# DARYL-GWZ/Proud-SLAM

Measured on AMD Instinct MI355X. Metric: rays/sec render+backward, Replica room0, 64 samples/ray, 1/2/4/8 MI355X, higher is better.
Workload: dtype f32

## Files before the change

### include/psvo.h

```cpp
#ifndef PSVO_H
#define PSVO_H

#include <stdint.h>

#ifdef __cplusplus
extern "C" {
#endif

enum {
    PSVO_OK = 0,
    PSVO_E_INVALID = 1,
    PSVO_E_LAUNCH = 2,
    PSVO_E_OVERFLOW = 3,
    PSVO_E_BUSY = 4,
    PSVO_E_SYSTEM = 5
};

const char *psvo_last_error(void);
const char *psvo_version(void);


int psvo_svo_intersect(void *stream, int b, int n, int m, float voxelsize, int n_max, const float *ray_start,
                       const float *ray_dir, const float *points, const int *children, int *idx, float *min_depth,
                       float *max_depth);
// ... 180 lines not shown
                          float voxel_size, int *table, int *row);
int psvo_mesh_depth_points(void *stream, int64_t n, const float *depth, const float *dirs, const float *pose,
                           double *out);
int64_t psvo_mesh_downsample_workspace_bytes(int64_t n);
int psvo_mesh_points_downsample(void *stream, int64_t n, const double *points, double cell, void *workspace,
                                double *out, int64_t *count);
int psvo_mesh_points_status(int64_t word);
int64_t psvo_mesh_ball_workspace_bytes(int64_t m);
int psvo_mesh_ball_any(void *stream, int64_t m, const double *points, int64_t n_verts, const float *verts,
                       double radius, void *workspace, uint8_t *hit, int64_t *status);

int psvo_adam_mark_rows(void *stream, int64_t m, const int *leaf, const int *vertex_idx, uint8_t *flags);
int psvo_adam_flags_from_state(void *stream, int64_t n_rows, const float *exp_avg, const float *exp_avg_sq,
                               uint8_t *flags);
int psvo_adam_step(void *stream, int n_tensors, float *const *params, const float *const *grads,
                   float *const *exp_avg, float *const *exp_avg_sq, const int64_t *numel, double lr, double beta1,
                   double beta2, double eps, double weight_decay, int64_t step);

typedef struct psvo_engine psvo_engine;

typedef struct psvo_map_desc {
    int64_t n_nodes;
    const float *centres;
    const int *structure;
    const int *vertex_idx;
    float *emb;
    int64_t n_emb;
    float *emb_m, *emb_v;
    float *dec[10];
    float *dec_m[10];
    float *dec_v[10];
    int width;
    float voxel_size, step_size, max_distance, truncation, max_depth;
    float w_rgb, w_depth, w_fs, w_sdf;
    double lr_emb, lr_dec, beta1, beta2, eps;
    float *grad_flat;
    const void *packed;
    uint8_t *emb_row_flags;
    uint8_t *emb_row_local;
} psvo_map_desc;

enum { PSVO_STEP_NO_ADAM = 1, PSVO_STEP_NO_LOSS = 4 };

int64_t psvo_map_grad_floats(int64_t n_emb);
int64_t psvo_map_grad_floats_w(int64_t n_emb, int width);

typedef struct psvo_pixel_frame {
    const float *dirs;
    const float *rgb;
    const float *depth;
    uint8_t *mask;
} psvo_pixel_frame;
int64_t psvo_sample_pixels_workspace_ints(int n_frames, int64_t n_pix);
int psvo_sample_pixels(void *stream, int n_frames, int64_t n_pix, int64_t k, const float *weights, int joint_sum,
                       const float *u, uint64_t seed, const psvo_pixel_frame *frames, int *workspace, int64_t *idx,
                       float *out_dirs, float *out_rgb, float *out_depth);

int64_t psvo_rows_workspace_ints(int64_t n_rows);
int psvo_rows_compact(void *stream, int64_t n_rows, int width, const float *grad, int *workspace, int *ids,
                      float *rows, int *count);
int psvo_rows_scatter_add(void *stream, int64_t n_list, int width, const int *ids, const float *rows, float *grad);
int psvo_rows_compact_flagged(void *stream, int64_t n_rows, int width, const float *grad, const uint8_t *flags,
                              int *workspace, int *ids, float *rows, int *count);
int psvo_rows_clear(void *stream, int64_t n_list, int width, const int *ids, float *grad, uint8_t *flags);
int psvo_rows_mark(void *stream, int64_t n_list, const int *ids, uint8_t *flags);
int psvo_rows_flags_from_grad(void *stream, int64_t n_rows, int width, const float *grad, uint8_t *flags);

psvo_engine *psvo_engine_new(void);
void psvo_engine_free(psvo_engine *e);
enum { PSVO_XCH_GATHER_I32 = 1, PSVO_XCH_SUM_I32 = 2, PSVO_XCH_SUM_F64 = 3, PSVO_XCH_QUERY = 0x100 };
typedef int (*psvo_exchange_fn)(void *user, int op, int64_t in_off, int64_t out_off, int64_t count, void *stream);
int64_t psvo_engine_exchange_words(int world, int64_t max_rays_global, int64_t max_rays_rank);
int psvo_engine_set_exchange(psvo_engine *e, int rank, int world, int64_t max_rays_global, int64_t max_rays_rank,
                             psvo_exchange_fn fn, void *user, int *xi32, double *xf64);

int psvo_engine_queued(psvo_engine *e);
int psvo_map_discard(psvo_engine *e);

enum {
    PSVO_PATH_QUERY_SPLIT = 1,
    PSVO_PATH_PADDED = 2,
    PSVO_PATH_DENSE_DECODER = 4,
    PSVO_PATH_INTERP_PASS = 8,
    PSVO_PATH_BWD_TWO_LAUNCH = 16
};
int psvo_engine_set_paths(psvo_engine *e, int paths);

int psvo_engine_select_stats(psvo_engine *e, void *stream, int64_t *out, int reset);

int psvo_engine_gate_stream(psvo_engine *e, void *stream);

int psvo_debug_set_lookback(int mask, int spin_bound, int delay_us);
int psvo_debug_set_bwd_split(int cost_a, int cost_b, int cost_b0);
int psvo_debug_bwd_split(int64_t units_a, int64_t units_b, int n_wg);
int psvo_debug_lb_helps(int64_t *out3, int reset);
int psvo_debug_set_pixel_draw(int mode);
int psvo_debug_select_samples(void *stream, int64_t r_hit, int s_max, float truncation, float max_depth,
                              const int *offsets, const int *ray_ns, const float *z_vals, int z_stride,
                              const int *rank_ray, const float *gt_depth, const float *sdf_s, const float *feat,
                              const int *leaf, const float *t, const int *ray_of, int64_t cap, int split, int *cidx,
                              int *offa, int *offb, float *feat_c, int *leaf_c, float *t_c, int *ray_of_c,
                              float *rgb_c, int *src_c, int *counts, uint64_t *desc, uint32_t tag, int *host_flag);
int64_t psvo_debug_select_granules(int64_t r_hit);
int psvo_debug_trunk_interp(void *stream, int fused, int64_t m_cap, const int *m_dev, const int *leaf, const float *t,
                            const int *ray_of, const int *ray_index, const float *rays_o, const float *rays_d,
                            const float *centres, const int *vertex_idx, const float *emb, float voxel_size,
                            const float *w1, const float *b1, const float *w2, const float *b2, const float *w3,
                            const float *b3, const float *w4, const float *b4, const float *w5, const float *b5,
                            float *images, float *sdf, float *h2, float *feat);
int psvo_debug_composite_loss(void *stream, int64_t r_hit, int s_max, float truncation, float max_depth,
                              const int *offsets, const int *ray_ns, const float *z_vals, int z_stride,
                              const int *rank_ray, const float *gt_rgb, const float *gt_depth, const float *sdf_s,
                              const float *rgb_s, const float *coef, float *workspace, float *color, float *depth,
                              float *grad_sdf_s, float *grad_rgb_s, int partials, const int *cidx);

enum { PSVO_TIME_MLP_FWD = 0, PSVO_TIME_MLP_BWD = 1, PSVO_TIME_INTERP_FWD = 2, PSVO_TIME_INTERP_BWD = 3,
       PSVO_TIME_INTERSECT = 4, PSVO_TIME_SAMPLE = 5, PSVO_TIME_POINTS = 6, PSVO_TIME_SELECT = 7,
       PSVO_TIME_REGIONS = 8 };
int psvo_engine_set_timing(psvo_engine *e, int on);
int psvo_engine_timing(psvo_engine *e, double *mean_ms);
int psvo_engine_set_clock(psvo_engine *e, int max_steps);
int psvo_engine_clock(psvo_engine *e, double *period_ms, int *n_steps);
int psvo_host_wait_stats(double *wait_us, long long *calls, long long *waited, int reset);

int psvo_map_query(psvo_engine *e, void *stream, const psvo_map_desc *d, int64_t n_rays, const float *rays_o,
                   const float *rays_d, uint64_t seed);
int psvo_map_step(psvo_engine *e, void *stream, const psvo_map_desc *d, int64_t n_rays, const float *rays_o,
                  const float *rays_d, const float *gt_rgb, const float *gt_depth, uint64_t seed, int64_t adam_step,
                  int flags, float *loss_out, int *stats_out);

typedef struct psvo_map_frames {
    int n_frames;
    int64_t rays_per_frame;
    const float *dirs_cam;
    float *poses, *pose_m, *pose_v;
    const int64_t *pose_step;
    double lr_pose;
    float *pose_grad;
    const float *next_dirs_cam;
    uint64_t next_seed;
    void *next_stream;
    const float *next_gt_depth;
} psvo_map_frames;
int psvo_map_step_frames(psvo_engine *e, void *stream, const psvo_map_desc *d, const psvo_map_frames *frames,
                         const float *gt_rgb, const float *gt_depth, const float *noise, uint64_t seed,
                         int64_t adam_step, int flags, float *loss_out, int *stats_out);

enum { PSVO_TRACK_DEPTH_FILTER = 2 };
int psvo_track_step(psvo_engine *e, void *stream, const psvo_map_desc *d, int64_t n_rays, const float *dirs_cam,
                    const float *gt_rgb, const float *gt_depth, float *pose, float *pose_m, float *pose_v, double lr,
                    const float *noise, uint64_t seed, int64_t adam_step, int flags, float *pose_grad,
                    float *loss_out, int *stats_out);

enum { PSVO_ADAM_ROWS_EXCHANGED = 1 };
int psvo_map_adam(psvo_engine *e, void *stream, const psvo_map_desc *d, int64_t adam_step);
int psvo_map_adam_ex(psvo_engine *e, void *stream, const psvo_map_desc *d, int64_t adam_step, int flags);
int psvo_map_join(psvo_engine *e, void *stream);
int psvo_map_side_wait(psvo_engine *e, void *stream);
int psvo_engine_grad_rays(psvo_engine *e, void *stream, int64_t n_rays, float *grad_o, float *grad_d);

typedef struct psvo_render_opts {
    int64_t tile_rays;
    int flags;
} psvo_render_opts;
enum { PSVO_RENDER_QUERY_ONLY = 1 };
enum {
    PSVO_RENDER_STAT_R_HIT = 0,
    PSVO_RENDER_STAT_P = 1,
    PSVO_RENDER_STAT_MAX_STEPS = 2,
// ... 78 lines not shown
```

### proud-slam_amd/csrc/composite.hip

```cpp
#include <hip/hip_runtime.h>

#include "lookback.h"
#include "psvo_common.h"
#include "query.h"
#include "select_common.h"

namespace psvo {
namespace {

__device__ __forceinline__ float wsum(float v) {
#pragma unroll
    for (int s = 32; s > 0; s >>= 1) v += __shfl_xor(v, s, 64);
    return v;
}
__device__ __forceinline__ int wmin(int v) {
#pragma unroll
    for (int s = 32; s > 0; s >>= 1) v = min(v, __shfl_xor(v, s, 64));
    return v;
}
__device__ __forceinline__ float sigm(float x) { return 1.0f / (1.0f + expf(-x)); }

__device__ __forceinline__ float comp_gw3(float gdp, float z, float gwx, bool has_c, float c0, float c1, float c2,
                                          float gr, float gg, float gb) {
    const float g = fmaf(gdp, z, gwx);
    return has_c ? fmaf(gb, c2, fmaf(gg, c1, fmaf(gr, c0, g))) : g;
}
__device__ __forceinline__ float comp_gw(float gdp, float z, float gwx, const float *c, float gr, float gg, float gb) {
    return c ? comp_gw3(gdp, z, gwx, true, c[0], c[1], c[2], gr, gg, gb) : comp_gw3(gdp, z, gwx, false, 0.f, 0.f,
                                                                                   0.f, gr, gg, gb);
}
__device__ __forceinline__ float comp_gsdf_sig(float gw, float dot, float tot, bool keep, float sp, float sn, float tr,
                                               float g) {
    const float gu = keep ? (gw - dot) / tot : 0.f;
    const float du = sp * sn * (sn - sp) / tr;
    return fmaf(gu, du, g);
}
__device__ __forceinline__ float comp_gsdf(float gw, float dot, float tot, bool keep, float sdf, float tr, float g) {
    const float a = sdf / tr;
    return comp_gsdf_sig(gw, dot, tot, keep, sigm(a), sigm(-a), tr, g);
}

__global__ __launch_bounds__(256) void k_composite_fwd(int64_t r_hit, int s_max, float tr,
                                                       const int *__restrict__ offsets,
                                                       const int *__restrict__ ray_ns,
                                                       const float *__restrict__ z_vals,
                                                       const float *__restrict__ sdf_s,
                                                       const float *__restrict__ rgb_s, float *__restrict__ sdf,
                                                       float *__restrict__ weights, float *__restrict__ color,
                                                       float *__restrict__ depth, float *__restrict__ z_min_out) {
    const int lane = threadIdx.x & 63;
    const int64_t r = (int64_t)blockIdx.x * (blockDim.x >> 6) + (threadIdx.x >> 6);
    if (r >= r_hit) return;
    const int off = offsets[r], ns = ray_ns[r];
    const float *z = z_vals + r * s_max;
    float *sd = sdf + r * s_max;
    float *wt = weights + r * s_max;
    int first = s_max;
    for (int s = lane; s < s_max; s += 64) {
        const float v = s < ns ? sdf_s[off + s] : 1.0f;
        sd[s] = v;
        if (s + 1 < s_max) {
            const float v1 = (s + 1) < ns ? sdf_s[off + s + 1] : 1.0f;
            if (v1 * v < 0.0f) first = min(first, s);
        }
    }
    first = wmin(first);
    const int ind = first == s_max ? 0 : first;
    const float zmin = z[ind];
    float tot = 0.f;
    for (int s = lane; s < s_max; s += 64) {
        const float v = sd[s];
        const float a = v / tr;
        float w = sigm(a) * sigm(-a);
        const bool keep = (z[s] < zmin + tr) && (s < ns);
        w = keep ? w : 0.0f;
        wt[s] = w;
        tot += w;
    }
    tot = wsum(tot) + 1e-8f;
    float cr = 0.f, cg = 0.f, cb = 0.f, dd = 0.f;
    for (int s = lane; s < s_max; s += 64) {
        const float w = wt[s] / tot;
        wt[s] = w;
        if (s < ns) {
            const float *c = rgb_s + (int64_t)(off + s) * 3;
            cr += w * c[0];
            cg += w * c[1];
            cb += w * c[2];
        }
        dd += w * z[s];
    }
    cr = wsum(cr);
    cg = wsum(cg);
    cb = wsum(cb);
    dd = wsum(dd);
    if (lane == 0) {
        color[r * 3 + 0] = cr;
        color[r * 3 + 1] = cg;
        color[r * 3 + 2] = cb;
        depth[r] = dd;
        if (z_min_out) z_min_out[r] = zmin;
    }
}

__global__ __launch_bounds__(256) void k_composite_bwd(int64_t r_hit, int s_max, float tr,
                                                       const int *__restrict__ offsets,
                                                       const int *__restrict__ ray_ns,
                                                       const float *__restrict__ z_vals,
                                                       const float *__restrict__ sdf,
                                                       const float *__restrict__ weights,
                                                       const float *__restrict__ rgb_s,
                                                       const float *__restrict__ g_color,
                                                       const float *__restrict__ g_depth,
                                                       const float *__restrict__ g_weights,
                                                       const float *__restrict__ g_sdf,
                                                       float *__restrict__ g_sdf_s, float *__restrict__ g_rgb_s) {
    const int lane = threadIdx.x & 63;
    const int64_t r = (int64_t)blockIdx.x * (blockDim.x >> 6) + (threadIdx.x >> 6);
    if (r >= r_hit) return;
    const int off = offsets[r], ns = ray_ns[r];
    const float *z = z_vals + r * s_max;
    const float *sd = sdf + r * s_max;
    const float *wt = weights + r * s_max;
    const float gr = g_color ? g_color[r * 3 + 0] : 0.f;
    const float gg = g_color ? g_color[r * 3 + 1] : 0.f;
    const float gb = g_color ? g_color[r * 3 + 2] : 0.f;
    const float gdp = g_depth ? g_depth[r] : 0.f;
    float dot = 0.f, tot = 0.f;
    for (int s = lane; s < s_max; s += 64) {
        const float gw = comp_gw(gdp, z[s], g_weights ? g_weights[r * s_max + s] : 0.f,
                                 s < ns ? rgb_s + (int64_t)(off + s) * 3 : nullptr, gr, gg, gb);
        dot = fmaf(gw, wt[s], dot);
    }
    dot = wsum(dot);
    int first = s_max;
    for (int s = lane; s < s_max; s += 64) {
        if (s + 1 < s_max && sd[s + 1] * sd[s] < 0.0f) first = min(first, s);
    }
    first = wmin(first);
    const float zmin = z[first == s_max ? 0 : first];
    for (int s = lane; s < s_max; s += 64) {
        const float a = sd[s] / tr;
        const bool keep = (z[s] < zmin + tr) && (s < ns);
        tot += keep ? sigm(a) * sigm(-a) : 0.f;
    }
    tot = wsum(tot) + 1e-8f;
    for (int s = lane; s < ns; s += 64) {
        const float *c = rgb_s + (int64_t)(off + s) * 3;
        const float W = wt[s];
        const float gw = comp_gw(gdp, z[s], g_weights ? g_weights[r * s_max + s] : 0.f, c, gr, gg, gb);
        g_sdf_s[off + s] = comp_gsdf(gw, dot, tot, z[s] < zmin + tr, sd[s], tr, g_sdf ? g_sdf[r * s_max + s] : 0.f);
        float *gc = g_rgb_s + (int64_t)(off + s) * 3;
        gc[0] = W * gr;
        gc[1] = W * gg;
        gc[2] = W * gb;
    }
}

constexpr int kPartColor = 0, kPartDepth = 1, kPartQFs = 5, kPartQSdf = 6, kPartN = 8;

struct CritTerms {
    float f, sm, xfs, ysdf;
};
__device__ __forceinline__ CritTerms crit_terms(float z, float p, float d, float tr, float max_depth) {
#pragma clang fp contract(off)
    CritTerms o;
    o.f = z < (d - tr) ? 1.0f : 0.0f;
    const float b = z > (d + tr) ? 1.0f : 0.0f;
    const float dm = (d > 0.0f && d < max_depth) ? 1.0f : 0.0f;
    o.sm = (1.0f - o.f) * (1.0f - b) * dm;
    o.xfs = p * o.f - o.f;
    o.ysdf = (z + p * tr) * o.sm - d * o.sm;
    return o;
}
__device__ __forceinline__ float crit_sq_add(float acc, float x) {
#pragma clang fp contract(off)
    return acc + x * x;
}
__device__ __forceinline__ float crit_grad(float cfs, float csdf, const CritTerms &t) {
#pragma clang fp contract(off)
    return cfs * t.xfs * t.f + csdf * t.ysdf * t.sm;
}

template <int J>
__global__ __launch_bounds__(256) void k_composite_loss(int64_t r_hit, int s_max, float tr, float max_depth,
                                                        const int *__restrict__ offsets,
                                                        const int *__restrict__ ray_ns,
                                                        const float *__restrict__ z_vals, int z_stride,
                                                        const int *__restrict__ rank_ray,
                                                        const float *__restrict__ gt_rgb,
                                                        const float *__restrict__ gt_depth,
                                                        const float *__restrict__ sdf_s,
                                                        const float *__restrict__ rgb_s,
                                                        const float *__restrict__ coef, float *__restrict__ part,
                                                        float *__restrict__ color, float *__restrict__ depth,
                                                        float *__restrict__ g_sdf_s, float *__restrict__ g_rgb_s,
                                                        int partials, const int *__restrict__ cidx) {
    const int lane = threadIdx.x & 63;
    const int64_t r = (int64_t)blockIdx.x * (blockDim.x >> 6) + (threadIdx.x >> 6);
    if (r >= r_hit) return;
    const int64_t orig = rank_ray[r];
    const int off = offsets[r], ns = ray_ns[r];
    const int lim = ns < s_max ? ns : s_max;
    const float d = gt_depth[orig];
    const float gt0 = gt_rgb[orig * 3 + 0], gt1 = gt_rgb[orig * 3 + 1], gt2 = gt_rgb[orig * 3 + 2];
    const float ccol = coef[0], cdep = coef[1], cfs = coef[2], csdf = coef[3];
    const float *z = z_vals + r * z_stride;
    auto z_at = [&](int s) { return s < ns ? z[s] : kMaxDepthFill; };
    auto sdf_at = [&](int s) { return s < ns ? sdf_s[off + s] : 1.0f; };
    auto ci_at = [&](int s) { return s < ns ? (cidx ? cidx[off + s] : off + s) : -1; };
    constexpr int JR = J > 0 ? J : 1;
    float zr[JR], pr[JR], c0r[JR], c1r[JR], c2r[JR];
    if constexpr (J > 0) {
#pragma unroll
        for (int j = 0; j < J; ++j) {
            const int s = lane + 64 * j;
            zr[j] = s < s_max ? z_at(s) : 0.f;
            pr[j] = sdf_at(s);
            const int ci = ci_at(s);
            const bool v = ci >= 0;
            const float *c = rgb_s + (int64_t)(v ? ci : 0) * 3;
            c0r[j] = v ? c[0] : 0.f;
            c1r[j] = v ? c[1] : 0.f;
            c2r[j] = v ? c[2] : 0.f;
        }
    }
    auto Z = [&](int j, int s) {
        if constexpr (J > 0) return zr[j]; else return z_at(s);
    };
    auto P = [&](int j, int s) {
        if constexpr (J > 0) return pr[j]; else return sdf_at(s);
    };
    auto C = [&](int j, int s, int k) {
        if constexpr (J > 0) return k == 0 ? c0r[j] : (k == 1 ? c1r[j] : c2r[j]);
        else {
            const int ci = ci_at(s);
            return ci >= 0 ? rgb_s[(int64_t)ci * 3 + k] : 0.f;
        }
    };
#define PSVO_FOR_S(lim) for (int j = 0, s = lane; (J == 0 || j < J) && s < (lim); ++j, s += 64)
    float pn[JR];
    if constexpr (J > 0) {
#pragma unroll
        for (int j = 0; j < J; ++j) {
            const float dn = __shfl_down(pr[j], 1, 64);
            const float nx = __shfl(pr[j + 1 < J ? j + 1 : j], 0, 64);
            pn[j] = lane < 63 ? dn : nx;
        }
    }
    int first = s_max;
    PSVO_FOR_S(lim) {
        const float v = P(j, s);
        float v1;
        if constexpr (J > 0) v1 = pn[j];
        else v1 = s + 1 < s_max ? sdf_at(s + 1) : 0.f;
        if (s + 1 < s_max && v1 * v < 0.0f) first = min(first, s);
    }
    first = wmin(first);
    const float zmin = z_at(first == s_max ? 0 : first);
    float spr[JR], snr[JR], wr[JR];
#pragma unroll
    for (int j = 0; j < JR; ++j) spr[j] = snr[j] = wr[j] = 0.f;
    float tot = 0.f;
    PSVO_FOR_S(lim) {
        const float a = P(j, s) / tr;
        const float sp = sigm(a), sn = sigm(-a);
        float w = sp * sn;
        const bool keep = (Z(j, s) < zmin + tr) && (s < ns);
        tot += keep ? w : 0.0f;
        if constexpr (J > 0) {
            spr[j] = sp;
            snr[j] = sn;
            wr[j] = keep ? w : 0.0f;
        }
    }
    tot = wsum(tot) + 1e-8f;
    if constexpr (J > 0) {
#pragma unroll
        for (int j = 0; j < J; ++j) wr[j] = wr[j] / tot;
    }
    auto weight_at = [&](int j, int s) {
        if constexpr (J > 0) {
            return wr[j];
        } else {
            const float a = P(j, s) / tr;
            const float w = sigm(a) * sigm(-a);
            const bool keep = (Z(j, s) < zmin + tr) && (s < ns);
            return (keep ? w : 0.0f) / tot;
        }
    };
    float cr = 0.f, cg = 0.f, cb = 0.f, dd = 0.f;
    PSVO_FOR_S(lim) {
        const float w = weight_at(j, s);
        if (s < ns) {
            cr += w * C(j, s, 0);
            cg += w * C(j, s, 1);
            cb += w * C(j, s, 2);
        }
        dd += w * Z(j, s);
    }
    cr = wsum(cr);
    cg = wsum(cg);
    cb = wsum(cb);
    dd = wsum(dd);
    float qfs = 0.f, qsdf = 0.f;
    if (partials) {
        PSVO_FOR_S(s_max) {
            const CritTerms t = crit_terms(Z(j, s), P(j, s), d, tr, max_depth);
            qfs = crit_sq_add(qfs, t.xfs);
            qsdf = crit_sq_add(qsdf, t.ysdf);
        }
        qfs = wsum(qfs);
        qsdf = wsum(qsdf);
    }
    const float rgb[3] = {cr, cg, cb};
    const float gt[3] = {gt0, gt1, gt2};
    float gcol[3], ac = 0.f;
#pragma unroll
    for (int c = 0; c < 3; ++c) {
        const float e = gt[c] - rgb[c];
        ac += fabsf(e);
        gcol[c] = -ccol * (e > 0.0f ? 1.0f : (e < 0.0f ? -1.0f : 0.0f));
    }
    const bool valid = d > 0.01f && d < max_depth;
    const float ed = d - dd;
    const float gdp = valid ? -cdep * (ed > 0.0f ? 1.0f : (ed < 0.0f ? -1.0f : 0.0f)) : 0.0f;
    if (lane == 0) {
        color[r * 3 + 0] = cr;
        color[r * 3 + 1] = cg;
        color[r * 3 + 2] = cb;
        depth[r] = dd;
        if (partials) {
            float *o = part + r * kPartN;
            o[kPartColor] = ac;
            o[kPartDepth] = valid ? fabsf(ed) : 0.0f;
            o[kPartQFs] = qfs;
            o[kPartQSdf] = qsdf;
            o[7] = 0.0f;
        }
    }
    float dot = 0.f;
    PSVO_FOR_S(lim) {
        const bool v = s < ns;
        const float gw = comp_gw3(gdp, Z(j, s), 0.f, v, v ? C(j, s, 0) : 0.f, v ? C(j, s, 1) : 0.f,
                                  v ? C(j, s, 2) : 0.f, gcol[0], gcol[1], gcol[2]);
        dot = fmaf(gw, weight_at(j, s), dot);
    }
    dot = wsum(dot);
    PSVO_FOR_S(ns) {
        const float W = weight_at(j, s);
        const float zs = Z(j, s);
        const float gw = comp_gw3(gdp, zs, 0.f, true, C(j, s, 0), C(j, s, 1), C(j, s, 2), gcol[0], gcol[1], gcol[2]);
        const float p = P(j, s);
        const float gsdf = crit_grad(cfs, csdf, crit_terms(zs, p, d, tr, max_depth));
        const int gi = ci_at(s);
        if (gi < 0) continue;
        if constexpr (J > 0)
            g_sdf_s[gi] = comp_gsdf_sig(gw, dot, tot, zs < zmin + tr, spr[j], snr[j], tr, gsdf);
        else
            g_sdf_s[gi] = comp_gsdf(gw, dot, tot, zs < zmin + tr, p, tr, gsdf);
        float *gc = g_rgb_s + (int64_t)gi * 3;
        gc[0] = W * gcol[0];
        gc[1] = W * gcol[1];
        gc[2] = W * gcol[2];
    }
#undef PSVO_FOR_S
}


constexpr int kSelWaves = 8, kSelMaxRpw = 16;
struct SelectArgs {
    const float4 *feat;
    const int *leaf, *ray_of;
    const float *t;
    int *cidx;
    int *offa, *offb;
    float4 *feat_c;
    int *leaf_c, *ray_of_c;
    float *t_c;
    float *rgb_c;
    int *src_c;
    int64_t cap;
    int split;
    int *counts;
    unsigned long long *desc;
    uint32_t tag;
    LbCtl ctl;
    int *host_flag;
};

using sel::sel_zmin;

struct SelFlags {
    bool keep, comp;
};
__device__ __forceinline__ SelFlags sel_flags(float zs, float zmin, float d, float tr, float max_depth) {
#pragma clang fp contract(off)
    SelFlags o;
    o.comp = zs < zmin + tr;
    const bool f = zs < (d - tr);
    const bool b = zs > (d + tr);
    const bool dm = d > 0.0f && d < max_depth;
    o.keep = o.comp || f || (!b && dm);
    return o;
}

__device__ unsigned long long psvo_g_sel_helps;

__global__ __launch_bounds__(512) void k_select_samples(int64_t r_hit, int rpw, int s_max, float tr, float max_depth,
                                                        const int *__restrict__ offsets,
                                                        const int *__restrict__ ray_ns,
                                                        const float *__restrict__ z_vals, int z_stride,
                                                        const int *__restrict__ rank_ray,
                                                        const float *__restrict__ gt_depth,
                                                        const float *__restrict__ sdf_s, SelectArgs a) {
    __shared__ int s_na[kSelWaves * kSelMaxRpw], s_nb[kSelWaves * kSelMaxRpw];
    __shared__ int s_oa[kSelWaves * kSelMaxRpw], s_ob[kSelWaves * kSelMaxRpw];
    __shared__ float s_zmin[kSelWaves * kSelMaxRpw];
    __shared__ int s_nc[kSelWaves], s_base[2];
    const int lane = threadIdx.x & 63, w = threadIdx.x >> 6;
    const int blk = (int)blockIdx.x;
    lb_debug_delay(a.ctl, blk);
    if (threadIdx.x == 0) lb_mark_started<3>(a.desc, blk, (int)gridDim.x, a.tag);
    const int64_t r0 = ((int64_t)blk * kSelWaves + w) * rpw;
    const uint64_t below = (1ull << lane) - 1ull;
    const bool split = a.split != 0;
    auto count_classes = [&](int cur) {
        const int64_t c0 = ((int64_t)cur * kSelWaves + w) * rpw;
        int nc_w = 0;
        for (int k = 0; k < rpw; ++k) {
            const int64_t r = c0 + k;
            int na = 0, nb = 0;
            float zmin = 0.f;
            if (r < r_hit) {
                const int off = offsets[r], ns = ray_ns[r];
                const float *z = z_vals + r * z_stride;
                const float d = gt_depth[rank_ray[r]];
                zmin = sel_zmin(lane, s_max, ns, off, z, sdf_s);
                for (int s0 = 0; s0 < ns; s0 += 64) {
                    const int s = s0 + lane;
                    SelFlags f{false, false};
                    if (s < ns) f = sel_flags(z[s], zmin, d, tr, max_depth);
                    const int nk = __popcll(__ballot(f.keep)), nc = __popcll(__ballot(f.comp && s < ns));
                    na += split ? nc : nk;
                    nb += split ? nk - nc : 0;
                    nc_w += nc;
                }
            }
            if (lane == 0) {
                s_na[w * rpw + k] = na;
                s_nb[w * rpw + k] = nb;
// ... 109 lines not shown
            a.offa[r] = ba;
            if (split) a.offb[r] = bb;
        }
        for (int s0 = 0; s0 < ns; s0 += 64) {
            const int s = s0 + lane;
            SelFlags f{false, false};
            if (s < ns) f = sel_flags(z[s], zmin, d, tr, max_depth);
            const bool in_a = split ? (f.comp && s < ns) : f.keep;
            const bool in_b = split && f.keep && !f.comp;
            const uint64_t bal_a = __ballot(in_a), bal_b = __ballot(in_b);
            const int64_t j = in_a ? (int64_t)(ba + __popcll(bal_a & below))
                                   : a.cap + bb + __popcll(bal_b & below);
            if (s < ns) a.cidx[off + s] = (in_a || in_b) ? (int)j : -1;
            if (in_a || in_b) {
                const int64_t src = off + s;
                a.leaf_c[j] = a.leaf[src];
                a.t_c[j] = a.t[src];
                a.ray_of_c[j] = a.ray_of[src];
                if (a.src_c) a.src_c[j] = (int)src;
                if (a.feat_c) {
#pragma unroll
                    for (int q = 0; q < 4; ++q) a.feat_c[j * 4 + q] = a.feat[src * 4 + q];
                }
                if (in_b) {
#pragma unroll
                    for (int k = 0; k < 3; ++k) a.rgb_c[j * 3 + k] = 0.f;
                }
            }
            ba += __popcll(bal_a);
            bb += __popcll(bal_b);
        }
    }
}

}
}

using namespace psvo;

extern "C" int psvo_composite_fwd(void *stream, int64_t r_hit, int s_max, float truncation, const int *offsets,
                                  const int *ray_ns, const float *z_vals, const float *sdf_s, const float *rgb_s,
                                  float *sdf, float *weights, float *color, float *depth, float *z_min) {
    PSVO_REQUIRE(r_hit >= 0 && s_max > 0 && truncation > 0.f, "composite_fwd: bad sizes");
    if (r_hit == 0) return PSVO_OK;
    psvo::launch(k_composite_fwd, dim3(div_up(r_hit, 4)), dim3(256), 0, as_stream(stream), r_hit, s_max,
                       truncation, offsets, ray_ns, z_vals, sdf_s, rgb_s, sdf, weights, color, depth, z_min);
    return check_launch("composite_fwd");
}

extern "C" int psvo_composite_bwd(void *stream, int64_t r_hit, int s_max, float truncation, const int *offsets,
                                  const int *ray_ns, const float *z_vals, const float *sdf, const float *weights,
                                  const float *rgb_s, const float *grad_color, const float *grad_depth,
                                  const float *grad_weights, const float *grad_sdf, float *grad_sdf_s,
                                  float *grad_rgb_s) {
    PSVO_REQUIRE(r_hit >= 0 && s_max > 0 && truncation > 0.f, "composite_bwd: bad sizes");
    if (r_hit == 0) return PSVO_OK;
    psvo::launch(k_composite_bwd, dim3(div_up(r_hit, 4)), dim3(256), 0, as_stream(stream), r_hit, s_max,
                       truncation, offsets, ray_ns, z_vals, sdf, weights, rgb_s, grad_color, grad_depth,
                       grad_weights, grad_sdf, grad_sdf_s, grad_rgb_s);
    return check_launch("composite_bwd");
}


extern "C" int psvo_composite_loss(void *stream, int64_t r_hit, int s_max, float truncation, float max_depth,
                                   const int *offsets, const int *ray_ns, const float *z_vals, const int *rank_ray,
                                   const float *gt_rgb, const float *gt_depth, const float *sdf_s,
                                   const float *rgb_s, const float *coef, float *workspace, float *color,
                                   float *depth, float *grad_sdf_s, float *grad_rgb_s) {
    return psvo::composite_loss_z(stream, r_hit, s_max, truncation, max_depth, offsets, ray_ns, z_vals, s_max,
                                  rank_ray, gt_rgb, gt_depth, sdf_s, rgb_s, coef, workspace, color, depth, grad_sdf_s,
                                  grad_rgb_s, true, nullptr);
}

int psvo::composite_loss_z(void *stream, int64_t r_hit, int s_max, float truncation, float max_depth,
                           const int *offsets, const int *ray_ns, const float *z_vals, int z_stride,
                           const int *rank_ray, const float *gt_rgb, const float *gt_depth, const float *sdf_s,
                           const float *rgb_s, const float *coef, float *workspace, float *color, float *depth,
                           float *grad_sdf_s, float *grad_rgb_s, bool partials, const int *cidx) {
    PSVO_REQUIRE(r_hit >= 0 && s_max > 0 && truncation > 0.f && z_stride >= s_max, "composite_loss: bad sizes");
    PSVO_REQUIRE(offsets && ray_ns && z_vals && rank_ray && gt_rgb && gt_depth && sdf_s && rgb_s && coef &&
                     workspace && color && depth && grad_sdf_s && grad_rgb_s,
                 "composite_loss: null pointer");
    if (r_hit == 0) return PSVO_OK;
    auto kern = s_max <= 128   ? k_composite_loss<2>
                : s_max <= 256 ? k_composite_loss<4>
                : s_max <= 512 ? k_composite_loss<8>
                               : k_composite_loss<0>;
    psvo::launch(kern, dim3(div_up(r_hit, 4)), dim3(256), 0, as_stream(stream), r_hit, s_max, truncation,
                       max_depth, offsets, ray_ns, z_vals, z_stride, rank_ray, gt_rgb, gt_depth, sdf_s, rgb_s, coef,
                       workspace, color, depth, grad_sdf_s, grad_rgb_s, partials ? 1 : 0, cidx);
    return check_launch("composite_loss");
}

int psvo::select_samples(hipStream_t st, int64_t r_hit, int s_max, float truncation, float max_depth,
                         const int *offsets, const int *ray_ns, const float *z_vals, int z_stride, const int *rank_ray,
                         const float *gt_depth, const float *sdf_s, const float *feat, const int *leaf, const float *t,
                         const int *ray_of, int64_t cap, bool split, int *cidx, int *offa, int *offb, float *feat_c,
                         int *leaf_c, float *t_c, int *ray_of_c, float *rgb_c, int *src_c, int *counts,
                         unsigned long long *desc, uint32_t tag, int *host_flag) {
    PSVO_REQUIRE(r_hit >= 0 && s_max > 0 && truncation > 0.f && z_stride >= s_max && tag != 0 && cap > 0,
                 "select_samples: bad sizes");
    PSVO_REQUIRE(!split || (offb != nullptr && rgb_c != nullptr),
                 "select_samples: the split needs class B's offsets and colour rows");
    const int rpw = select_rays_per_wave(r_hit);
    PSVO_REQUIRE(rpw <= kSelMaxRpw, "select_samples: %lld hit rays exceed the selection's %d",
                 (long long)r_hit, kSelWaves * kSelMaxRpw * kLbMaxBlocks);
    if (r_hit == 0) return PSVO_OK;
    SelectArgs a{reinterpret_cast<const float4 *>(feat), leaf, ray_of, t, cidx, offa, offb,
                 reinterpret_cast<float4 *>(feat_c), leaf_c, ray_of_c, t_c, rgb_c, src_c, cap, split ? 1 : 0, counts, desc, tag,
                 lb_ctl(4), host_flag};
    psvo::launch(k_select_samples, dim3(div_up(r_hit, (int64_t)kSelWaves * rpw)), dim3(64 * kSelWaves), 0, st, r_hit,
                 rpw, s_max, truncation, max_depth, offsets, ray_ns, z_vals, z_stride, rank_ray, gt_depth, sdf_s, a);
    return check_launch("select_samples");
}

int psvo::lb_helps_select(int64_t *out1, bool reset) {
    unsigned long long h = 0;
    if (hipDeviceSynchronize() != hipSuccess || hipMemcpyFromSymbol(&h, HIP_SYMBOL(psvo_g_sel_helps), sizeof(h)) != hipSuccess)
        return set_error(PSVO_E_LAUNCH, "debug_lb_helps: copy failed");
    *out1 = (int64_t)h;
    const unsigned long long z = 0;
    if (reset && hipMemcpyToSymbol(HIP_SYMBOL(psvo_g_sel_helps), &z, sizeof(z)) != hipSuccess)
        return set_error(PSVO_E_LAUNCH, "debug_lb_helps: reset failed");
    return PSVO_OK;
}

int psvo::select_rays_per_wave(int64_t r_hit) {
    const int64_t per = (int64_t)kSelWaves * kLbMaxBlocks;
    return r_hit <= per ? 1 : (int)((r_hit + per - 1) / per);
}

int64_t psvo::select_granules(int64_t r_hit) {
    return lb_granules<3>(div_up(r_hit, (int64_t)kSelWaves * select_rays_per_wave(r_hit)));
}
```

### proud-slam_amd/csrc/engine.cpp

```cpp
#include <stdio.h>
#include <stdlib.h>
#include <string.h>

#include <utility>

#include "engine_internal.h"

namespace psvo {
RenderWs *&engine_render_ws(psvo_engine *e) { return e->render; }
bool engine_data_parallel(const psvo_engine *e) { return e->x.on(); }
}

using namespace psvo;
using namespace psvo::eng;

namespace psvo {
thread_local KernelClock *g_kclock = nullptr;

namespace eng {

void *arena_buf(Arena &a, hipStream_t st, int slot, size_t bytes, int *rc) {
    if (bytes == 0) bytes = 16;
    if (a.cap[slot] >= bytes) return a.p[slot];
    if (a.p[slot]) {
// ... 143 lines not shown
        return set_error(PSVO_E_LAUNCH, "engine: aux stream creation failed");
    for (hipEvent_t *ev : evs)
        if (hipEventCreateWithFlags(ev, (ev == &e->dfeat_ready ? 0 : hipEventDisableTiming) |
                                            hipEventDisableSystemFence) != hipSuccess)
            return set_error(PSVO_E_LAUNCH, "engine: event creation failed");
    return PSVO_OK;
}

void dec_sizes(int W, int64_t (&n)[10]) {
    const int64_t w = W;
    const int64_t v[10] = {w * 16, w, w * w, w, 129 * w, 129, w * 144, w, 3 * w, 3};
    for (int i = 0; i < 10; ++i) n[i] = v[i];
}

int map_adam(hipStream_t st, const psvo_map_desc *d, float *grads, int64_t adam_step, const PoseAdam *pa,
             bool sparse_rows) {
    constexpr int kMax = 11 + kXchMaxFrames;
    float *p[kMax];
    const float *g[kMax];
    float *m[kMax], *v[kMax];
    int64_t n[kMax], steps[kMax];
    double lr[kMax];
    int zero[kMax];
    const uint8_t *rows[kMax] = {};
    if (sparse_rows) rows[0] = d->emb_row_flags;
    p[0] = d->emb;
    g[0] = grads;
    m[0] = d->emb_m;
    v[0] = d->emb_v;
    n[0] = d->n_emb * 16;
    lr[0] = d->lr_emb;
    zero[0] = 1;
    int64_t off = d->n_emb * 16;
    int64_t kDecSizes[10];
    dec_sizes(d->width, kDecSizes);
    for (int i = 0; i < 10; ++i) {
        p[1 + i] = d->dec[i];
        g[1 + i] = grads + off;
        m[1 + i] = d->dec_m[i];
        v[1 + i] = d->dec_v[i];
        n[1 + i] = kDecSizes[i];
        lr[1 + i] = d->lr_dec;
        zero[1 + i] = 0;
        off += kDecSizes[i];
    }
    int cnt = 11;
    for (int i = 0; i < cnt; ++i) steps[i] = adam_step;
    for (int f = 0; pa && f < pa->n; ++f, ++cnt) {
        p[cnt] = pa->p[f];
        g[cnt] = pa->g[f];
        m[cnt] = pa->m[f];
        v[cnt] = pa->v[f];
        n[cnt] = 6;
        lr[cnt] = pa->lr;
        zero[cnt] = 0;
        steps[cnt] = pa->step[f];
    }
    return adam_launch(st, cnt, p, g, m, v, n, lr, d->beta1, d->beta2, d->eps, 0.0, adam_step, zero, steps, rows);
}

int pose_adam(hipStream_t st, const psvo_map_desc *d, const PoseAdam &pa) {
    if (pa.n == 0) return PSVO_OK;
    int64_t n6[kXchMaxFrames];
    double lr[kXchMaxFrames];
    int zero[kXchMaxFrames];
    for (int k = 0; k < pa.n; ++k) {
        n6[k] = 6;
        lr[k] = pa.lr;
        zero[k] = 0;
    }
    return adam_launch(st, pa.n, pa.p, pa.g, pa.m, pa.v, n6, lr, d->beta1, d->beta2, d->eps, 0.0, 1, zero,
                       const_cast<int64_t *>(pa.step));
}

}
}

extern "C" psvo_engine *psvo_engine_new(void) {
    psvo_engine *e = new psvo_engine();
    const char *ipass = getenv("PSVO_INTERP_PASS");
    if (ipass && ipass[0] == '1') e->paths |= PSVO_PATH_INTERP_PASS;
    const char *two = getenv("PSVO_BWD_TWO_LAUNCH");
    if (two && two[0] == '1') e->paths |= PSVO_PATH_BWD_TWO_LAUNCH;
    for (auto &q : e->qs)
        if (query_set_init(q) != PSVO_OK) {
            psvo_engine_free(e);
            return nullptr;
        }
    return e;
}

static EngineExchange exchange_layout(int world, int64_t max_rays_global, int64_t max_rays_rank) {
    EngineExchange x;
    x.world = world;
    x.nch = dist_slot0_rows(max_rays_global) / kSamplerG;
    x.max_rays_rank = max_rays_rank > 0 ? max_rays_rank : max_rays_global;
    x.cw = dist_count_words((int)x.max_rays_rank);
    return x;
}

extern "C" int64_t psvo_engine_exchange_words(int world, int64_t max_rays_global, int64_t max_rays_rank) {
    if (world < 1 || max_rays_global < 1 || max_rays_rank < 0 || max_rays_rank > max_rays_global) return -1;
    const EngineExchange x = exchange_layout(world, max_rays_global, max_rays_rank);
    return x.table_off() + x.table_words();
}

extern "C" int psvo_engine_set_exchange(psvo_engine *e, int rank, int world, int64_t max_rays_global,
                                        int64_t max_rays_rank, psvo_exchange_fn fn, void *user, int *xi32,
                                        double *xf64) {
    PSVO_REQUIRE(e, "engine_set_exchange: null engine");
    PSVO_REQUIRE(world >= 1 && rank >= 0 && rank < world && max_rays_global >= 1 && max_rays_rank >= 0 &&
                     max_rays_rank <= max_rays_global,
                 "engine_set_exchange: bad rank %d / world %d / max_rays_global %lld / max_rays_rank %lld", rank,
                 world, (long long)max_rays_global, (long long)max_rays_rank);
    PSVO_REQUIRE(e->q_count == 0, "engine_set_exchange: queries are queued");
    PSVO_REQUIRE(!fn || (xi32 && xf64), "engine_set_exchange: exchange buffers required");
    e->x = exchange_layout(world, max_rays_global, max_rays_rank);
    e->x.fn = fn;
    e->x.user = user;
    e->x.rank = rank;
    e->x.xi32 = xi32;
    e->x.xf64 = xf64;
    return PSVO_OK;
}

extern "C" int psvo_engine_set_paths(psvo_engine *e, int paths) {
    PSVO_REQUIRE(e && (paths & ~(PSVO_PATH_QUERY_SPLIT | PSVO_PATH_PADDED | PSVO_PATH_DENSE_DECODER |
                               PSVO_PATH_INTERP_PASS | PSVO_PATH_BWD_TWO_LAUNCH)) == 0,
                 "engine_set_paths: bad arguments");
    PSVO_REQUIRE(e->q_count == 0, "engine_set_paths: queries are queued");
    e->paths = paths;
    return PSVO_OK;
}

extern "C" int psvo_engine_gate_stream(psvo_engine *e, void *stream) {
    PSVO_REQUIRE(e, "engine_gate_stream: null engine");
    e->draw_gate_used = true;
    if (!e->draw_gate_recorded) return PSVO_OK;
    return st_wait(as_stream(stream), e->draw_gate_ev, "engine_gate_stream");
}

extern "C" int psvo_engine_select_stats(psvo_engine *e, void *stream, int64_t *out, int reset) {
    PSVO_REQUIRE(e && out, "engine_select_stats: null argument");
    for (int i = 0; i < 5; ++i) out[i] = 0;
    if (!e->a.p[kSelCnt]) return PSVO_OK;
    hipStream_t st = as_stream(stream);
    int c[psvo::kSelCountInts];
    if (hipMemcpyAsync(c, e->a.p[kSelCnt], sizeof(c), hipMemcpyDeviceToHost, st) != hipSuccess ||
        hipStreamSynchronize(st) != hipSuccess)
        return set_error(PSVO_E_LAUNCH, "engine_select_stats: copy failed");
    unsigned long long u[3];
    memcpy(u, c + 4, sizeof(u));
    out[0] = (int64_t)c[0] + c[1];
    out[1] = c[3];
    out[2] = (int64_t)u[0];
    out[3] = (int64_t)u[1];
    out[4] = (int64_t)u[2];
    if (c[2] & psvo::kLbFlagTimeout) {
        ENG_CALL(zero_async(static_cast<int *>(e->a.p[kSelCnt]) + 2, sizeof(int), st, "engine_select_stats"));
        if (e->host_flags) *(volatile int *)e->host_flags = 0;
        e->sel_zero_gen = 0;
        return set_error(PSVO_E_LAUNCH, "engine_select_stats: a sample selection's look-back wait was abandoned");
    }
    if (reset)
        ENG_CALL(zero_async(static_cast<int *>(e->a.p[kSelCnt]) + 4, 6 * sizeof(int), st, "engine_select_stats"));
    return PSVO_OK;
}

extern "C" int psvo_engine_set_timing(psvo_engine *e, int on) {
    PSVO_REQUIRE(e, "engine_set_timing: null engine");
    EngineTimer &t = e->tm;
    const char *mk = getenv("PSVO_TIMING_MARKERS");
    if (on && !t.ev[0][0])
        for (int r = 0; r < PSVO_TIME_REGIONS; ++r)
            for (int k = 0; k < 2; ++k)
                if (hipEventCreateWithFlags(&t.ev[r][k], hipEventReleaseToDevice) != hipSuccess)
                    return set_error(PSVO_E_LAUNCH, "engine_set_timing: hipEventCreate failed");
    const unsigned kc_flags = hipEventReleaseToDevice;
    if (on && !t.kc.ev[0][0])
        for (int i = 0; i < psvo::KernelClock::kMax; ++i)
            for (int k = 0; k < 2; ++k)
                if (hipEventCreateWithFlags(&t.kc.ev[i][k], kc_flags) != hipSuccess)
                    return set_error(PSVO_E_LAUNCH, "engine_set_timing: hipEventCreate failed");
    timer_collect(e, true);
    if (psvo::g_kclock == &t.kc) psvo::g_kclock = nullptr;
    t.kc.depth = 0;
    t.kc.overflow = false;
    t.on = on != 0;
    t.overlap = on == 2;
    t.markers = mk && *mk == '1';
    const char *ks = getenv("PSVO_TIMING_SPAN");
    t.kc.sum = !(ks && *ks == '1');
    t.kc.n = 0;
    t.kc.n_inst = 0;
    for (int r = 0; r < PSVO_TIME_REGIONS; ++r) {
        t.ms[r] = 0.0;
        t.n[r] = 0;
        t.kms[r] = 0.0;
        t.starts[r] = 0;
    }
    return PSVO_OK;
}

extern "C" int psvo_engine_timing(psvo_engine *e, double *mean_ms) {
    PSVO_REQUIRE(e && mean_ms, "engine_timing: null argument");
    EngineTimer &t = e->tm;
    timer_collect(e, true);
    for (int r = 0; r < PSVO_TIME_REGIONS; ++r) {
        if (t.markers)
            mean_ms[r] = t.n[r] ? t.ms[r] / (double)t.n[r] : -1.0;
        else
// ... 114 lines not shown
```

### proud-slam_amd/csrc/engine_internal.h

```cpp
#pragma once

#include <hip/hip_runtime.h>
#include <stdint.h>
#include <time.h>

#include <vector>

#include "psvo_common.h"
#include "lookback.h"
#include "query.h"

namespace psvo {

enum QSlot { kStats, kHitIdx, kHitT0, kHitT1, kRayNv, kRayDsum, kRayRank, kRankRay, kSIdx, kSDepth, kSDist, kRayNs,
             kOffsets, kBlkOut, kRayCnt, kCoefQ, kLbDesc, kLeafQ, kTQ, kRayOfQ, kDistSums, kMDev, kNvRank, kCol0Rank,
             kQSlots };
enum Slot {
    kLeaf, kT, kRayOf, kZ, kMask, kFeat, kImages, kSdfS, kRgbS, kAct, kMasks, kSdf, kWeights, kColor,
    kDepth, kZmin, kCritWs, kSums, kGLoss, kGColor, kGDepth, kGSdf, kGSdfS, kGRgbS, kMlpWs, kDfeat, kDecGrad,
    kGradEmb, kGradOD, kRaysO, kRaysD, kDTmp, kPoseGrad, kSumsC, kCoef, kIbWs,
    kCidx, kOffB, kFeatB, kLeafB, kTB, kRayOfB, kSdfB, kSelCnt, kSelDesc,
    kOffB2, kH2, kSrcC, kSlots
};

// ... 23 lines not shown
    const float *ro = nullptr, *rd = nullptr;
    const float *dirs = nullptr;
    const float *counts_gt = nullptr;
    uint64_t seed = 0;
    int max_steps = 0;
    hipEvent_t p1 = nullptr;
    hipEvent_t done2 = nullptr;
    bool p2_pending = false;
    const float *p2_gt = nullptr;
    float p2_tr = 0.f, p2_max_depth = 0.f;
};

}

struct EngineTimer {
    bool on = false;
    bool overlap = false;
    bool pending = false;
    bool markers = false;
    unsigned used = 0;
    hipEvent_t ev[PSVO_TIME_REGIONS][2] = {};
    double ms[PSVO_TIME_REGIONS] = {};
    int64_t n[PSVO_TIME_REGIONS] = {};
    psvo::KernelClock kc;
    double kms[PSVO_TIME_REGIONS] = {};
    int64_t starts[PSVO_TIME_REGIONS] = {};
};

struct EngineExchange {
    psvo_exchange_fn fn = nullptr;
    void *user = nullptr;
    int rank = 0, world = 1;
    int nch = 1;
    int cw = 8;
    int64_t max_rays_rank = 0;
    int *xi32 = nullptr;
    double *xf64 = nullptr;
    bool on() const { return fn != nullptr; }
    int64_t in_off() const { return 0; }
    int64_t all_off() const { return cw; }
    int64_t q2_in_off() const { return all_off() + (int64_t)world * cw; }
    int64_t q2_all_off() const { return q2_in_off() + psvo::kDistWordsPerRank; }
    int64_t table_off() const { return (q2_all_off() + (int64_t)world * psvo::kDistWordsPerRank + 63) / 64 * 64; }
    int64_t table_words() const { return (int64_t)psvo::kSamplerG * nch; }
    int call(int op, int64_t in, int64_t out, int64_t count, hipStream_t st, const char *what) const {
        const int rc = fn(user, op, in, out, count, st);
        if (rc != 0) return psvo::set_error(PSVO_E_LAUNCH, "exchange (%s) failed with %d", what, rc);
        return PSVO_OK;
    }
};

struct EngineClock {
    std::vector<hipEvent_t> ev;
    int n = 0;
    bool on = false;
};

struct psvo_engine {
    EngineExchange x;
    EngineClock clk;
    psvo::Arena a;
    psvo::QuerySet qs[2];
    int q_head = 0, q_count = 0;
    uint32_t lb_tag = 0;
    hipStream_t side = nullptr;
    hipStream_t q2s = nullptr;
    hipEvent_t in_ready = nullptr;
    hipStream_t aux = nullptr;
    hipStream_t lossq = nullptr;
    hipEvent_t dfeat_ready = nullptr, emb_done = nullptr, z_ready = nullptr, coef_ready = nullptr,
               grads_ready = nullptr, prep_fork = nullptr, prep_done = nullptr, loss_done = nullptr;
    hipEvent_t adam_done = nullptr;
    bool bwd_recorded = false;
    bool adam_pending = false;
    hipEvent_t next_ready = nullptr;
    hipEvent_t draw_gate = nullptr;
    hipEvent_t draw_gate_ev = nullptr;
    bool draw_gate_recorded = false;
    bool draw_gate_used = false;
    EngineTimer tm;
    bool images_next = false;
    const float *images_w0 = nullptr;
    int paths = 0;
    int64_t m_early = 0;
    uint32_t sel_tag = 0;
    uint32_t sel_zero_gen = 0;
    int *host_flags = nullptr;
    bool grads_clean = false;
    const float *clean_buf = nullptr;
    psvo::RenderWs *render = nullptr;
};

#define ENG_CALL(x)                     \
    do {                                \
        const int _rc = (x);            \
        if (_rc != PSVO_OK) return _rc; \
    } while (0)

#define ENG_BUF(T, name, slot, bytes)                                              \
    T *name = reinterpret_cast<T *>(arena_buf(e->a, st, slot, (bytes), &rc));     \
    if (!name) return rc;
#define Q_BUF(T, name, slot, bytes)                                              \
    T *name = reinterpret_cast<T *>(arena_buf(q.a, st, slot, (bytes), &rc));    \
    if (!name) return rc;

#pragma GCC visibility push(hidden)
namespace psvo {
namespace eng {

inline int ev_record(hipEvent_t ev, hipStream_t st, const char *who) {
    if (hipEventRecord(ev, st) == hipSuccess) return PSVO_OK;
    return set_error(PSVO_E_LAUNCH, "%s: event record failed", who);
}
inline int st_wait(hipStream_t st, hipEvent_t ev, const char *who) {
    if (hipStreamWaitEvent(st, ev, 0) == hipSuccess) return PSVO_OK;
    return set_error(PSVO_E_LAUNCH, "%s: stream wait failed", who);
}
inline int zero_async(void *p, size_t bytes, hipStream_t st, const char *who) {
    if (hipMemsetAsync(p, 0, bytes, st) == hipSuccess) return PSVO_OK;
    return set_error(PSVO_E_LAUNCH, "%s: memset failed", who);
}
inline int fork_join(hipStream_t from, hipStream_t st, hipEvent_t ev) {
    if (from == st) return PSVO_OK;
    ENG_CALL(ev_record(ev, from, "engine"));
    return st_wait(st, ev, "engine");
}

inline double now_ns() {
    timespec t;
    clock_gettime(CLOCK_MONOTONIC, &t);
    return t.tv_sec * 1e9 + t.tv_nsec;
}

void *arena_buf(Arena &a, hipStream_t st, int slot, size_t bytes, int *rc);
void timer_collect(psvo_engine *e, bool block = false);
void mark(psvo_engine *e, hipStream_t st, int region, int end);
int join_adam(psvo_engine *e, hipStream_t st, const char *who, double host_wait_us = 0.0);
inline bool engine_overlap(psvo_engine *e) { return !e->tm.on || e->tm.overlap; }
int ensure_aux(psvo_engine *e);
void dec_sizes(int W, int64_t (&n)[10]);
struct PoseAdam {
    int n = 0;
    float *p[kXchMaxFrames], *m[kXchMaxFrames], *v[kXchMaxFrames];
    const float *g[kXchMaxFrames];
    int64_t step[kXchMaxFrames];
    double lr = 0.0;
};
int map_adam(hipStream_t st, const psvo_map_desc *d, float *grads, int64_t adam_step, const PoseAdam *pa = nullptr,
             bool sparse_rows = false);
int pose_adam(hipStream_t st, const psvo_map_desc *d, const PoseAdam &pa);

int query_set_init(QuerySet &s);
void query_set_free(QuerySet &s);
void host_wait_report();
int query_enqueue(psvo_engine *e, hipStream_t st, QuerySet &q, const psvo_map_desc *d, int64_t R,
                  const float *rays_o, const float *rays_d, uint64_t seed, const char *who,
                  const float *noise = nullptr, bool record_done = true, const float *counts_gt = nullptr);
int take_query(psvo_engine *e, hipStream_t st, const psvo_map_desc *d, int64_t R, const float *rays_o,
               const float *rays_d, uint64_t seed, const char *who, QuerySet **out, const float *noise = nullptr,
               const float *counts_gt = nullptr);
int freed_wait(QuerySet &q, hipStream_t s);
int release_query(psvo_engine *e, hipStream_t st, QuerySet *q);
struct QueryGuard {
    psvo_engine *e;
    hipStream_t st;
    QuerySet *q = nullptr;
// ... 23 lines not shown
```

### proud-slam_amd/csrc/engine_step.cpp

```cpp
#include <stdint.h>
#include <string.h>

#include <algorithm>

#include "engine_internal.h"
#include "interp_load.h"

using namespace psvo;
using namespace psvo::eng;

namespace {

struct Samples {
    int *offsets = nullptr, *leaf = nullptr, *ray_of = nullptr;
    float *tt = nullptr, *feat = nullptr, *rgb_s = nullptr, *act = nullptr;
    uint64_t *masks = nullptr;
};

struct Render {
    int64_t r_hit = 0, m = 0;
    int s_max = 0;
    int *rank_ray = nullptr, *ray_rank = nullptr, *ray_ns = nullptr;
    float *z_vals = nullptr, *images = nullptr, *sdf_s = nullptr;
    Samples s;
// ... 302 lines not shown
    ENG_BUF(float, g_sdf, kGSdf, RS * sizeof(float));
    ENG_CALL(psvo_criterion_bwd_ex(stream, r_hit, s_max, d->truncation, d->max_depth, q.rank_ray, gt_rgb, gt_depth,
                                   q.color, q.depth, q.sdf, q.z_vals, loss_out, g_loss, dtmp, dthr, g_color, g_depth,
                                   g_sdf));
    ENG_BUF(float, g_sdf_s, kGSdfS, M * sizeof(float));
    ENG_BUF(float, g_rgb_s, kGRgbS, M * 3 * sizeof(float));
    ENG_CALL(psvo_composite_bwd(stream, r_hit, s_max, d->truncation, q.s.offsets, q.ray_ns, q.z_vals, q.sdf, q.weights,
                                q.s.rgb_s, g_color, g_depth, nullptr, g_sdf, g_sdf_s, g_rgb_s));
    *g_sdf_s_out = g_sdf_s;
    *g_rgb_s_out = g_rgb_s;
    return PSVO_OK;
}

int frames_update(psvo_engine *e, hipStream_t st, const psvo_map_desc *d, const psvo_map_frames *fr,
                  const Render &q, const float *grad_od, int64_t R, PoseAdam *pa) {
    int rc = PSVO_OK;
    float *pg = fr->pose_grad;
    if (!pg) {
        ENG_BUF(float, gbuf, kPoseGrad, (size_t)fr->n_frames * 8 * sizeof(float));
        pg = gbuf;
    }
    ENG_CALL(psvo::pose_grad_frames_rays(st, fr->n_frames, fr->rays_per_frame, q.ray_rank, fr->dirs_cam, grad_od,
                                         grad_od + R * 3, fr->poses, pg));
    pa->n = 0;
    pa->lr = fr->lr_pose;
    for (int f = 0; f < fr->n_frames; ++f) {
        if (fr->pose_step[f] < 1) continue;
        const int k = pa->n++;
        pa->p[k] = fr->poses + f * 6;
        pa->m[k] = fr->pose_m + f * 6;
        pa->v[k] = fr->pose_v + f * 6;
        pa->g[k] = pg + f * 8;
        pa->step[k] = fr->pose_step[f];
    }
    return PSVO_OK;
}

int frames_lookahead(psvo_engine *e, hipStream_t st, const psvo_map_desc *d, const psvo_map_frames *fr,
                     int64_t R, const Render &cur, const float *grad_od, bool record_done) {
    int rc = PSVO_OK;
    PSVO_REQUIRE(e->q_count == 0, "map_step_frames: a query is already queued");
    QuerySet &q = e->qs[e->q_head];
    ENG_CALL(freed_wait(q, st));
    ENG_BUF(float, rays_o, kRaysO, (size_t)R * 3 * sizeof(float));
    ENG_BUF(float, rays_d, kRaysD, (size_t)R * 3 * sizeof(float));
    float *pg = fr->pose_grad;
    if (!pg) {
        ENG_BUF(float, gbuf, kPoseGrad, (size_t)fr->n_frames * 8 * sizeof(float));
        pg = gbuf;
    }
    ENG_CALL(psvo::pose_step_frames(st, fr->n_frames, fr->rays_per_frame, cur.ray_rank, fr->dirs_cam,
                                    grad_od, grad_od + R * 3, fr->poses, fr->pose_m, fr->pose_v, fr->pose_step,
                                    fr->lr_pose, d->beta1, d->beta2, d->eps, pg, fr->next_dirs_cam, rays_o, rays_d));
    ENG_CALL(query_enqueue(e, st, q, d, R, rays_o, rays_d, fr->next_seed, "map_step_frames (look-ahead)", nullptr,
                           record_done, fr->next_gt_depth));
    q.dirs = fr->next_dirs_cam;
    q.pending = true;
    e->q_count++;
    return PSVO_OK;
}

struct MapStep {
    psvo_engine *e;
    hipStream_t st;
    const psvo_map_desc *d;
    const psvo_map_frames *fr;
    int flags;
    int64_t R, adam_step;
    const float *rays_o, *rays_d, *gt_rgb, *gt_depth;
    float *loss_out;
    bool overlap = false, dist = false, want_loss = false, wait_next = false, ahead = false, split = false;
    hipStream_t ax = nullptr, lq = nullptr, eb = nullptr;
    const float *counts_gt = nullptr;
    uint8_t *mark_into = nullptr;
    bool sparse_rows = false;
    QuerySet *qset = nullptr;
    Render q;
    bool empty = false;
    int64_t n_hit = 0;
    Samples k;
    int *cidx = nullptr, *sel_cnt = nullptr, *offb = nullptr;
    const int *h2_src = nullptr;
    float *crit_ws = nullptr, *coef = nullptr, *g_sdf_s = nullptr, *g_rgb_s = nullptr;
    double *sums = nullptr;
    float *grads = nullptr, *grad_od = nullptr;
    float *G[10] = {};

    bool two_class() const { return q.sparse && d->width == 128; }
    int64_t m_rows() const { return q.sparse ? 2 * q.m : q.m; }
    bool join_loss() const { return want_loss && lq != ax; }
    bool no_adam() const { return (flags & PSVO_STEP_NO_ADAM) != 0; }
};

int step_select(MapStep &s) {
    psvo_engine *e = s.e;
    hipStream_t st = s.st;
    const psvo_map_desc *d = s.d;
    const Render &q = s.q;
    s.k = q.s;
    if (!q.sparse || s.empty) return PSVO_OK;
    int rc = PSVO_OK;
    const int64_t M = q.m, r_hit = q.r_hit;
    const int64_t M2 = 2 * M;
    ENG_BUF(int, cx, kCidx, M * sizeof(int));
    ENG_BUF(int, offa, kOffB, (size_t)(r_hit + 1) * sizeof(int));
    float *feat_c = nullptr;
    if (!q.h2) {
        ENG_BUF(float, fc, kFeatB, M2 * 16 * sizeof(float));
        feat_c = fc;
    }
    ENG_BUF(int, leaf_c, kLeafB, M2 * sizeof(int));
    ENG_BUF(float, t_c, kTB, M2 * sizeof(float));
    ENG_BUF(int, ray_of_c, kRayOfB, M2 * sizeof(int));
    ENG_BUF(int, cnt, kSelCnt, psvo::kSelCountInts * sizeof(int));
    ENG_BUF(unsigned long long, desc, kSelDesc, (size_t)psvo::select_granules(r_hit) * sizeof(unsigned long long));
    if (e->sel_zero_gen != e->a.gen[kSelDesc]) {
        ENG_CALL(zero_async(desc, e->a.cap[kSelDesc], st, "map_step"));
        ENG_CALL(zero_async(cnt, psvo::kSelCountInts * sizeof(int), st, "map_step"));
        e->sel_zero_gen = e->a.gen[kSelDesc];
    }
    if (!e->host_flags) {
        if (hipHostMalloc(reinterpret_cast<void **>(&e->host_flags), sizeof(int),
                          hipHostMallocCoherent | hipHostMallocMapped) != hipSuccess)
            return set_error(PSVO_E_LAUNCH, "map_step: pinned allocation failed");
        *e->host_flags = 0;
    }
    if (s.two_class()) {
        ENG_BUF(int, ob, kOffB2, (size_t)(r_hit + 1) * sizeof(int));
        s.offb = ob;
    }
    ENG_BUF(float, rgb_c, kRgbS, M2 * 3 * sizeof(float));
    int *src_c = nullptr;
    if (q.h2) {
        ENG_BUF(int, sc, kSrcC, M2 * sizeof(int));
        src_c = sc;
    }
    e->sel_tag = e->sel_tag == 0xffffffffu ? 1u : e->sel_tag + 1u;
    mark(e, st, PSVO_TIME_SELECT, 0);
    if (e->draw_gate_used && !e->draw_gate &&
        hipEventCreateWithFlags(&e->draw_gate, hipEventDisableSystemFence) != hipSuccess)
        return set_error(PSVO_E_LAUNCH, "map_step: event creation failed");
    {
        psvo::StopBind gate(e->draw_gate_used ? e->draw_gate : nullptr, true);
        const int sel_rc = psvo::select_samples(st, r_hit, q.s_max, d->truncation, d->max_depth, q.s.offsets, q.ray_ns,
                                                q.z_vals, q.z_stride, q.rank_ray, s.gt_depth, q.sdf_s, q.s.feat,
                                                q.s.leaf, q.s.tt, q.s.ray_of, M, s.two_class(), cx, offa, s.offb,
                                                feat_c, leaf_c, t_c, ray_of_c, rgb_c, src_c, cnt, desc, e->sel_tag,
                                                e->host_flags);
        if (gate.consumed() && gate.bound()) {
            e->draw_gate_ev = gate.bound();
            e->draw_gate_recorded = true;
        }
        ENG_CALL(sel_rc);
    }
    mark(e, st, PSVO_TIME_SELECT, 1);
    ENG_BUF(float, sdf_b, kSdfB, M * sizeof(float));
    ENG_BUF(float, act, kAct, (size_t)psvo_mlp_act_floats(M, d->width) * sizeof(float));
    ENG_BUF(uint64_t, masks, kMasks, (size_t)psvo_mlp_mask_words(M, d->width) * sizeof(uint64_t));
    const psvo::H2Rows h2r{nullptr, q.h2, src_c};
    float *feat_k = src_c ? q.s.feat : feat_c;
    ENG_CALL(mlp_fwd_prepared(st, M, d->width, feat_k, q.images, sdf_b, rgb_c, act, masks, cnt,
                              src_c ? &h2r : nullptr));
    mark(e, st, PSVO_TIME_MLP_FWD, 1);
    s.k = Samples{offa, leaf_c, ray_of_c, t_c, feat_k, rgb_c, act, masks};
    s.h2_src = src_c;
    s.cidx = cx;
    s.sel_cnt = cnt;
    return PSVO_OK;
}

int step_normalisers(MapStep &s) {
    psvo_engine *e = s.e;
    hipStream_t st = s.st, ax = s.ax;
    const psvo_map_desc *d = s.d;
    const Render &q = s.q;
    QuerySet *qset = s.qset;
    const EngineExchange &x = e->x;
    int rc = PSVO_OK;
    ENG_BUF(float, crit_ws, kCritWs, psvo_criterion_workspace_floats(q.r_hit) * sizeof(float));
    s.crit_ws = crit_ws;
    double *sums_c = x.xf64;
    s.sums = x.xf64 ? x.xf64 + 8 : nullptr;
    if (!s.dist) {
        ENG_BUF(double, sc, kSumsC, 8 * sizeof(double));
        ENG_BUF(double, sl, kSums, 8 * sizeof(double));
        sums_c = sc;
        s.sums = sl;
    }
    const bool coef_q = !s.dist && s.counts_gt && qset->counts_gt == s.counts_gt;
    const bool sums_q = s.dist && s.counts_gt && qset->counts_gt != nullptr &&
                        !(qset->host_stats[PSVO_STAT_FLAGS] & psvo::PSVO_FLAG_UNION_UNCOUNTED);
    s.coef = coef_q ? static_cast<float *>(qset->a.p[kCoefQ]) : nullptr;
    if (!coef_q) {
        ENG_BUF(float, cbuf, kCoef, 4 * sizeof(float));
        s.coef = cbuf;
    }
    if (s.dist) {
        if (sums_q) {
            sums_c = static_cast<double *>(qset->a.p[kDistSums]);
            ENG_CALL(st_wait(ax, qset->done2, "map_step"));
        } else {
            ENG_CALL(criterion_counts(ax, s.empty ? 0 : q.r_hit, q.s_max, d->truncation, d->max_depth, q.rank_ray,
                                      s.gt_depth, q.z_vals, q.z_stride, q.z_stride == q.s_max ? nullptr : q.ray_ns,
                                      crit_ws, sums_c));
            ENG_CALL(x.call(PSVO_XCH_SUM_F64, 0, 0, 8, ax, "loss normalisers"));
        }
        ENG_CALL(criterion_coef_from_sums(ax, sums_c, s.n_hit, q.s_max, d->truncation, d->w_rgb, d->w_depth, d->w_fs,
                                          d->w_sdf, kCritFlags, s.coef));
    } else if (!coef_q) {
        ENG_CALL(psvo::criterion_coef_z(ax, q.r_hit, q.s_max, d->truncation, d->max_depth, q.rank_ray, s.gt_depth,
                                        q.z_vals, q.z_stride, q.ray_ns, d->w_rgb, d->w_depth, d->w_fs, d->w_sdf,
                                        kCritFlags, crit_ws, sums_c, s.coef));
    }
    if (!coef_q) ENG_CALL(fork_join(ax, st, e->coef_ready));
    if (s.mark_into && !s.empty && !psvo::mlp_bwd_fuses_interp(d->width))
        ENG_CALL(psvo_adam_mark_rows(ax, q.m, q.s.leaf, d->vertex_idx, s.mark_into));
    return PSVO_OK;
}

int step_loss(MapStep &s) {
    psvo_engine *e = s.e;
    hipStream_t st = s.st, lq = s.lq;
    const psvo_map_desc *d = s.d;
    const Render &q = s.q;
    int rc = PSVO_OK;
    ENG_BUF(float, color, kColor, (size_t)q.r_hit * 3 * sizeof(float));
    ENG_BUF(float, depth, kDepth, (size_t)q.r_hit * sizeof(float));
    ENG_BUF(float, g_sdf_s, kGSdfS, s.m_rows() * sizeof(float));
    ENG_BUF(float, g_rgb_s, kGRgbS, s.m_rows() * 3 * sizeof(float));
    s.g_sdf_s = g_sdf_s;
    s.g_rgb_s = g_rgb_s;
    if (!s.empty)
        ENG_CALL(psvo::composite_loss_z(st, q.r_hit, q.s_max, d->truncation, d->max_depth, q.s.offsets, q.ray_ns,
                                        q.z_vals, q.z_stride, q.rank_ray, s.gt_rgb, s.gt_depth, q.sdf_s, s.k.rgb_s,
                                        s.coef, s.crit_ws, color, depth, g_sdf_s, g_rgb_s, s.want_loss || s.dist,
                                        s.cidx));
    if (!s.want_loss) return PSVO_OK;
    ENG_CALL(fork_join(st, lq, e->grads_ready));
    if (!s.empty)
        ENG_CALL(psvo_criterion_reduce(lq, q.r_hit, s.crit_ws, s.sums));
    else
        ENG_CALL(zero_async(s.sums, 8 * sizeof(double), lq, "map_step"));
    if (s.dist) ENG_CALL(e->x.call(PSVO_XCH_SUM_F64, 8, 8, 8, lq, "loss sums"));
    ENG_CALL(psvo_criterion_finalize(lq, s.sums, s.n_hit, q.s_max, d->w_rgb, d->w_depth, d->w_fs, d->w_sdf,
                                     d->truncation, kCritFlags, s.loss_out));
    if (lq != s.ax) ENG_CALL(ev_record(e->loss_done, lq, "map_step"));
    return PSVO_OK;
}

int step_grad_buffers(MapStep &s) {
    psvo_engine *e = s.e;
    hipStream_t st = s.st;
    int rc = PSVO_OK;
    s.grads = s.d->grad_flat;
    if (!s.grads) {
        ENG_BUF(float, gbuf, kDecGrad, psvo_map_grad_floats_w(s.d->n_emb, s.d->width) * sizeof(float));
        s.grads = gbuf;
    }
    int64_t sizes[10];
    dec_sizes(s.d->width, sizes);
    int64_t off = s.d->n_emb * 16;
    for (int i = 0; i < 10; ++i) {
        s.G[i] = s.grads + off;
        off += sizes[i];
    }
    ENG_BUF(float, grad_od, kGradOD, (size_t)s.R * 6 * sizeof(float));
    s.grad_od = grad_od;
    return PSVO_OK;
}

int step_clock(psvo_engine *e, hipStream_t on) {
    if (e->clk.on && e->clk.n < (int)e->clk.ev.size()) ENG_CALL(ev_record(e->clk.ev[e->clk.n++], on, "map_step"));
    return PSVO_OK;
}

int step_empty(MapStep &s, QueryGuard &guard) {
    psvo_engine *e = s.e;
    ENG_CALL(fork_join(s.ax, s.st, e->emb_done));
    ENG_CALL(zero_async(s.grads, (size_t)psvo_map_grad_floats_w(s.d->n_emb, s.d->width) * sizeof(float), s.st,
                        "map_step"));
    e->grads_clean = false;
    ENG_CALL(guard.release());
    if (!s.no_adam()) ENG_CALL(map_adam(s.st, s.d, s.grads, s.adam_step));
    return step_clock(e, s.st);
}

int step_backward(MapStep &s) {
    psvo_engine *e = s.e;
    hipStream_t st = s.st, ax = s.ax, eb = s.eb;
    const psvo_map_desc *d = s.d;
    const Render &q = s.q;
    const Samples &k = s.k;
    int rc = PSVO_OK;
    const int64_t M = q.m, R = s.R;
    const int n_split = 256;
    ENG_BUF(float, mlp_ws, kMlpWs, psvo_mlp_workspace_floats_w(M, d->width, n_split) * sizeof(float));
    ENG_BUF(float, dfeat, kDfeat, M * 16 * sizeof(float));
    const bool fuse_ib = psvo::mlp_bwd_fuses_interp(d->width);
    float *grad_emb = s.grads;
    const size_t emb_bytes = (size_t)d->n_emb * 16 * sizeof(float);
    const bool emb_dirty = !(e->grads_clean && e->clean_buf == grad_emb);
    if (fuse_ib && emb_dirty) ENG_CALL(zero_async(grad_emb, emb_bytes, st, "map_step"));
    float *gx = nullptr;
    if (fuse_ib) {
        ENG_BUF(float, gxb, kIbWs, (size_t)s.m_rows() * 3 * sizeof(float));
        gx = gxb;
    }
    const psvo::InterpFuse ipf{k.leaf,  k.ray_of,      q.rank_ray, d->vertex_idx, k.tt, s.rays_o, s.rays_d, d->centres,
                               d->emb,  d->voxel_size, grad_emb,   gx,            s.mark_into};
    mark(e, st, PSVO_TIME_MLP_BWD, 0);
    const psvo::InterpFuse ipf_b{k.leaf + M, k.ray_of + M, q.rank_ray, d->vertex_idx, k.tt + M, s.rays_o, s.rays_d,
                                 d->centres, d->emb, d->voxel_size, grad_emb, gx ? gx + 3 * M : nullptr, s.mark_into};
    const psvo::TrunkBwd tbw{s.sel_cnt ? s.sel_cnt + 1 : nullptr, s.g_sdf_s + M, s.h2_src ? k.feat : k.feat + M * 16,
                             fuse_ib ? &ipf_b : nullptr, s.h2_src ? q.h2 : nullptr, s.h2_src ? s.h2_src + M : nullptr,
                             (e->paths & PSVO_PATH_BWD_TWO_LAUNCH) != 0};
    ENG_CALL(mlp_bwd(st, M, d->width, k.feat, q.images, k.rgb_s, k.act, k.masks, s.g_sdf_s, s.g_rgb_s, dfeat, s.G, 0,
                     n_split, mlp_ws, s.overlap ? e->dfeat_ready : nullptr, fuse_ib ? &ipf : nullptr,
                     s.split ? ax : nullptr, s.sel_cnt, s.two_class() ? &tbw : nullptr, s.h2_src));
    mark(e, st, PSVO_TIME_MLP_BWD, 1);
    if (s.overlap) e->bwd_recorded = true;
    if (s.overlap && eb != st) ENG_CALL(st_wait(eb, e->dfeat_ready, "map_step"));
    if (!fuse_ib && emb_dirty) ENG_CALL(zero_async(grad_emb, emb_bytes, eb, "map_step"));
    e->grads_clean = false;
    e->clean_buf = grad_emb;
    mark(e, eb, PSVO_TIME_INTERP_BWD, 0);
    if (fuse_ib) {
        ENG_CALL(psvo::interp_rays_gx(eb, q.r_hit, k.offsets, q.rank_ray, k.tt, gx, s.grad_od, s.grad_od + R * 3,
                                      s.two_class() ? s.offb : nullptr, s.two_class() ? k.tt + M : nullptr,
                                      s.two_class() ? gx + 3 * M : nullptr));
    } else {
        ENG_BUF(float, ib_ws2, kIbWs, psvo_interp_bwd_workspace_floats(q.r_hit, q.s_max) * sizeof(float));
        ENG_CALL(psvo_interp_bwd_chunked(eb, q.r_hit, q.s_max, 16, d->voxel_size, k.offsets, q.rank_ray, k.leaf, k.tt,
                                         s.rays_o, s.rays_d, d->centres, d->vertex_idx, d->emb, dfeat, grad_emb,
                                         s.grad_od, s.grad_od + R * 3, ib_ws2));
    }
    mark(e, eb, PSVO_TIME_INTERP_BWD, 1);
    if (s.overlap && eb != st) {
        ENG_CALL(ev_record(e->emb_done, eb, "map_step"));
        ENG_CALL(st_wait(st, e->emb_done, "map_step"));
    }
    if (s.join_loss()) ENG_CALL(st_wait(s.split ? ax : st, e->loss_done, "map_step"));
    return PSVO_OK;
}

int step_tail(MapStep &s) {
    psvo_engine *e = s.e;
    hipStream_t st = s.st, ax = s.ax, eb = s.eb;
    const psvo_map_desc *d = s.d;
    int rc = PSVO_OK;
    PoseAdam pa;
    if (s.ahead) {
        if (s.wait_next) ENG_CALL(st_wait(eb, e->next_ready, "map_step"));
        ENG_CALL(frames_lookahead(e, eb, d, s.fr, s.R, s.q, s.grad_od, eb != st));
    } else if (s.fr) {
        ENG_CALL(frames_update(e, st, d, s.fr, s.q, s.grad_od, s.R, &pa));
    }
    hipStream_t os = st;
    if (!s.no_adam()) {
        if (s.split) os = ax;
        ENG_CALL(map_adam(os, d, s.grads, s.adam_step, &pa, s.sparse_rows));
        e->grads_clean = true;
        if (s.ahead) {
            ENG_BUF(float, images, kImages, psvo_mlp_image_floats_w(d->width) * sizeof(float));
            ENG_CALL(mlp_images(os, d->width, d->dec, images));
            e->images_next = true;
            e->images_w0 = d->dec[0];
        }
        if (s.split) {
            ENG_CALL(ev_record(e->adam_done, ax, "map_step"));
            e->adam_pending = true;
        }
    } else {
        ENG_CALL(pose_adam(st, d, pa));
    }
    ENG_CALL(step_clock(e, os));
    if (s.split && s.join_loss()) ENG_CALL(st_wait(st, e->loss_done, "map_step"));
    return PSVO_OK;
}

int map_step_impl(psvo_engine *e, hipStream_t st, const psvo_map_desc *d, int64_t n_rays, const float *rays_o,
                  const float *rays_d, const float *gt_rgb, const float *gt_depth, const float *noise, uint64_t seed,
                  int64_t adam_step, int flags, float *loss_out, int *stats_out, const psvo_map_frames *fr) {
    PSVO_REQUIRE(e && d && rays_o && rays_d && gt_rgb && gt_depth && loss_out, "map_step: null argument");
    PSVO_REQUIRE(n_rays > 0 && adam_step >= 1, "map_step: bad sizes");
    PSVO_REQUIRE(d->width == 128 || d->width == 256, "map_step: decoder width %d unsupported (fused: 128, 256)",
                 d->width);
    MapStep s{e, st, d, fr, flags, n_rays, adam_step, rays_o, rays_d, gt_rgb, gt_depth, loss_out};
    s.want_loss = !(flags & PSVO_STEP_NO_LOSS);
    s.counts_gt = !s.want_loss ? gt_depth : nullptr;
    ENG_CALL(take_query(e, st, d, s.R, rays_o, rays_d, seed, "map_step", &s.qset, noise, s.counts_gt));
    QueryGuard guard{e, st, s.qset};
    s.overlap = engine_overlap(e);
    if (s.overlap) ENG_CALL(ensure_aux(e));
    s.dist = e->x.on();
    s.ax = s.overlap ? e->aux : st;
    s.lq = (s.overlap && !s.dist) ? e->lossq : s.ax;
    s.ahead = fr && fr->next_dirs_cam;
    s.split = psvo::mlp_bwd_split_tail(d->width) && s.overlap && s.ahead && !s.no_adam();
// ... 141 lines not shown
```

### proud-slam_amd/csrc/mlp128.h

```cpp
#pragma once
#include <hip/hip_runtime.h>

#include "psvo_common.h"

#ifdef PSVO_STAMPS
__device__ unsigned long long psvo_g_stamps[3][256][8][8][16];
#endif

namespace psvo {
namespace {

typedef float f32x16 __attribute__((ext_vector_type(16)));

constexpr int kW = 128;
constexpr int kIn = 16;
constexpr int kNB = kW / 32;

constexpr int kOffB1 = 0, kOffB2 = kOffB1 + 128, kOffB3 = kOffB2 + 128, kOffB4 = kOffB3 + 132,
              kOffB5 = kOffB4 + 128;
constexpr int kOffW3r0 = kOffB5 + 4, kOffW5 = kOffW3r0 + 128;
constexpr int kOffW = kOffW5 + 3 * 128;

constexpr int kF2Waves = 8, kF2Threads = kF2Waves * 64;

// ... 68 lines not shown
              kImgVec = kImgF4 + 18432,
              kVecPad = 1280,
              kImgC4 = kImgVec + kVecPad,
              kImgC3 = kImgC4 + 9 * 8 * 256,
              kImgC2 = kImgC3 + 8 * 8 * 256,
              kImgC1 = kImgC2 + 8 * 8 * 256,
              kImgT1 = kImgC1 + 8 * 256,
              kImgT2 = kImgT1 + 8 * 256,
              kImgTotal = kImgT2 + 8 * 8 * 256;
static_assert(kOffW <= kVecPad, "vector image");

__device__ __forceinline__ void raw_barrier() {
    asm volatile("" ::: "memory");
    __builtin_amdgcn_s_waitcnt(0xC07F);
    __builtin_amdgcn_s_barrier();
    asm volatile("" ::: "memory");
}

__device__ __forceinline__ float sigmoidf(float x) { return 1.0f / (1.0f + expf(-x)); }

__device__ __forceinline__ void load_x(const float *__restrict__ feat, int64_t s, bool valid, int h, float (&x)[8]) {
    const float *fr = feat + (valid ? s : 0) * kIn;
#pragma unroll
    for (int t = 0; t < 8; ++t) x[t] = valid ? fr[2 * t + h] : 0.0f;
}

__device__ __forceinline__ uint32_t lds_addr(const float *l) {
    return (uint32_t)(uintptr_t)(const __attribute__((address_space(3))) float *)l;
}
__device__ __forceinline__ void glds16(const float *g, float *l) {
    uint32_t keep;
    asm volatile("s_mov_b32 %0, m0\n\ts_mov_b32 m0, %2\n\ts_nop 0\n\tglobal_load_lds_dwordx4 %1, off\n\ts_mov_b32 m0, %0"
                 : "=&s"(keep)
                 : "v"(g), "s"(__builtin_amdgcn_readfirstlane(lds_addr(l)))
                 : "memory");
}

__device__ __forceinline__ void stage8(float *dst, const float *img, int n_floats, int wave, int lane) {
    for (int c = wave; c < n_floats / 256; c += kF2Waves) glds16(img + (c * 64 + lane) * 4, dst + c * 256);
}

__device__ __forceinline__ void store_nt(float *base, int i, float v) { __builtin_nontemporal_store(v, base + i); }

__device__ __forceinline__ void wait_vm(int n) {
    asm volatile("" ::: "memory");
    switch (n) {
        case 0: __builtin_amdgcn_s_waitcnt(0x0F70); break;
        case 1: __builtin_amdgcn_s_waitcnt(0x0F71); break;
        case 8: __builtin_amdgcn_s_waitcnt(0x0F78); break;
        case 9: __builtin_amdgcn_s_waitcnt(0x0F79); break;
        case 16: __builtin_amdgcn_s_waitcnt(0x4F70); break;
        case 17: __builtin_amdgcn_s_waitcnt(0x4F71); break;
        case 18: __builtin_amdgcn_s_waitcnt(0x4F72); break;
        default: __builtin_amdgcn_s_waitcnt(0x0F70); break;
    }
    asm volatile("" ::: "memory");
}

struct DwGrid {
    int wg_begin[5];
    int n_split[5];
    int slab_off[5];
    int slab_len[5];
};

struct DwDst {
    float *w[5], *b[5];
    int rows[5], cols[5];
    int elem_begin[6];
};

#ifdef PSVO_STAMPS
constexpr int kStampIters = 8, kStampWgs = 256;
#define PSVO_STAMP_DECL int stit_ = 0
#define PSVO_STAMP(i)                                                                               \
    do {                                                                                            \
        __builtin_amdgcn_sched_barrier(0);                                                          \
        const unsigned long long t_ = __builtin_amdgcn_s_memtime();                                 \
        __builtin_amdgcn_sched_barrier(0);                                                          \
        if ((threadIdx.x & 63) == 0 && stit_ < kStampIters && blockIdx.x < kStampWgs)               \
            psvo_g_stamps[kStampK][blockIdx.x][threadIdx.x >> 6][stit_][i] = t_;                         \
    } while (0)
#define PSVO_STAMP_FLUSH(k) ++stit_
#else
#define PSVO_STAMP_DECL
#define PSVO_STAMP(i)
#define PSVO_STAMP_FLUSH(k)
#endif

}
}
```

### proud-slam_amd/csrc/mlp_bwd.hip

```cpp
#include <hip/hip_runtime.h>

#include <cstdlib>

#include "interp_fuse.h"
#include "mlp128_chain16.h"
#include "mlp128_trunk_fb.h"
#include "psvo_common.h"

namespace psvo {
namespace {

constexpr int kDwRedEl = 64;
__device__ __forceinline__ float dw_sum_range(const float *__restrict__ p, int64_t stride, int b, int e) {
    float v = 0.0f;
    int sp = b;
    for (; sp + 8 <= e; sp += 8) {
        float q[8];
#pragma unroll
        for (int u = 0; u < 8; ++u) q[u] = p[(sp + u) * stride];
#pragma unroll
        for (int u = 0; u < 8; ++u) v += q[u];
    }
    for (; sp < e; ++sp) v += p[sp * stride];
    return v;
}
__global__ __launch_bounds__(256) void k_mlp_dw_reduce(DwGrid g, const float *__restrict__ slabs, DwDst dst,
                                                       int accumulate, const float *__restrict__ slabs_b,
                                                       const int *__restrict__ cnt, const int *__restrict__ cnt_b,
                                                       BwdSplitCost cost) {
    __shared__ float part[4][kDwRedEl];
    const int lane = threadIdx.x & 63, k = threadIdx.x >> 6;
    const int e = blockIdx.x * kDwRedEl + lane;
    const bool in = e < dst.elem_begin[5];
    int L = 0;
#pragma unroll
    for (int l = 1; l < 5; ++l) L += (e >= dst.elem_begin[l]);
    const int rel = in ? e - dst.elem_begin[L] : 0;
    const bool trunk_el = L < 2 || (L == 2 && (rel < 128 || rel == 129 * 128));
    int n_split = g.n_split[L];
    if (cnt) {
        const int64_t m_a = __builtin_amdgcn_readfirstlane(*cnt), m_b = __builtin_amdgcn_readfirstlane(*cnt_b);
        const int n_a = bwd_split_na((m_a + kU - 1) / kU, (m_b + kU - 1) / kU, n_split, cost);
        if (!trunk_el) n_split = n_a;
    }
    const int64_t stride = g.slab_len[L];
    const int b = n_split * k / 4, en = n_split * (k + 1) / 4;
    float v = 0.0f;
    if (in) {
        v = dw_sum_range(slabs + g.slab_off[L] + rel, stride, b, en);
        if (slabs_b && trunk_el) v += dw_sum_range(slabs_b + g.slab_off[L] + rel, stride, b, en);
    }
    part[k][lane] = v;
    __syncthreads();
    if (k != 0 || !in) return;
    v = ((part[0][lane] + part[1][lane]) + part[2][lane]) + part[3][lane];
    const int nw = dst.rows[L] * dst.cols[L];
    float *out = rel < nw ? dst.w[L] + rel : dst.b[L] + (rel - nw);
    *out = accumulate ? *out + v : v;
}

struct BwdIn16 {
    uint64_t mk[3];
    float y[3], g[3], gs;
    float4 x;
};

__device__ __forceinline__ void load_bwd_in16(const float *__restrict__ rgb_in, const uint64_t *__restrict__ masks,
                                              const float *__restrict__ g_sdf, const float *__restrict__ g_rgb,
                                              const float *__restrict__ feat, int64_t s, bool valid, int q,
                                              BwdIn16 &in, const int *__restrict__ x_src = nullptr) {
    const int64_t sv = valid ? s : 0;
    const uint64_t *mk = masks + (sv * 2 + (q & 1)) * 3;
#pragma unroll
    for (int i = 0; i < 3; ++i) {
        in.mk[i] = mk[i];
        in.y[i] = rgb_in[sv * 3 + i];
        in.g[i] = g_rgb[sv * 3 + i];
    }
    in.gs = g_sdf[sv];
    const int64_t xr = x_src ? (int64_t)x_src[sv] : sv;
    in.x = *reinterpret_cast<const float4 *>(feat + xr * kIn + 4 * q);
}

struct Bwd3Src {
    const float *rgb, *g_sdf, *g_rgb, *feat;
    const uint64_t *masks;
// ... 241 lines not shown
                *reinterpret_cast<float4 *>(page5) = p0;
                *reinterpret_cast<float4 *>(page5 + 4) = p1;
            }
            PSVO_STAMP(1);
            raw_barrier();
            PSVO_STAMP(2);
            if (r == n_rounds) break;
            dw_job<0, 0>(ring, eset(4 * r), nullptr, fm, ubase, true, h2m, ubase, true, u1, d, lane, acc4, b4p,
                         unused0, unused1);
            PSVO_STAMP(3);
            raw_barrier();
            PSVO_STAMP(4);
            dw_job<2, 2>(ring, eset(4 * r + 1), sset(r & 1) + 3 * kU, h2m, ubase, true, h1m, ubase, true, u1, d, lane, acc3, b3p,
                         r0, b30);
            PSVO_STAMP(5);
            raw_barrier();
            PSVO_STAMP(6);
            dw_job<0, 1>(ring, eset(4 * r + 2), nullptr, h1m, ubase, true, fm, ubase + 4, r + 1 < n_rounds, u1, d,
                         lane, acc2, b2p, unused0, unused1);
            PSVO_STAMP(7);
            raw_barrier();
            PSVO_STAMP(8);
            PSVO_STAMP_FLUSH(1);
        }
        const int rb[kNB] = {0, 1, 2, 3}, cb[1] = {d};
        float *s2 = slabs + g.slab_off[1] + (int64_t)b * g.slab_len[1];
        float *s3 = slabs + g.slab_off[2] + (int64_t)b * g.slab_len[2];
        float *s4 = slabs + g.slab_off[3] + (int64_t)b * g.slab_len[3];
        {
            f32x16 t[kNB][1];
#pragma unroll
            for (int k = 0; k < kNB; ++k) t[k][0] = acc2[k];
            dw_store<kNB, 1, true>(s2, 128, 0, 128, rb, cb, t, lane);
#pragma unroll
            for (int k = 0; k < kNB; ++k) t[k][0] = acc3[k];
            dw_store<kNB, 1, true>(s3, 128, 1, 128, rb, cb, t, lane);
#pragma unroll
            for (int k = 0; k < kNB; ++k) t[k][0] = acc4[k];
            dw_store<kNB, 1, true>(s4, 144, 0, 144, rb, cb, t, lane);
        }
        const float v2 = b2p + __shfl_xor(b2p, 32, 64), v3 = b3p + __shfl_xor(b3p, 32, 64),
                    v4 = b4p + __shfl_xor(b4p, 32, 64), vr0 = r0 + __shfl_xor(r0, 32, 64),
                    v30 = b30 + __shfl_xor(b30, 32, 64);
        if (h == 0) {
            store_nt(s2, 128 * 128 + 32 * d + i, v2);
            store_nt(s3, 129 * 128 + 1 + 32 * d + i, v3);
            store_nt(s4, 128 * 144 + 32 * d + i, v4);
            store_nt(s3, 32 * d + i, vr0);
        }
        if (d == 0 && lane == 0) store_nt(s3, 129 * 128, v30);
        float *s5 = slabs + g.slab_off[4] + (int64_t)b * g.slab_len[4];
        const float4 p0 = *reinterpret_cast<const float4 *>(page5), p1 = *reinterpret_cast<const float4 *>(page5 + 4);
        const float w5[3] = {p0.x, p0.y, p0.z}, b5[3] = {p1.x, p1.y, p1.z};
        float v5[3], t5[3];
#pragma unroll
        for (int ch = 0; ch < 3; ++ch) {
            v5[ch] = w5[ch] + __shfl_xor(w5[ch], 32, 64);
            t5[ch] = b5[ch] + __shfl_xor(b5[ch], 32, 64);
        }
        if (h == 0) {
#pragma unroll
            for (int ch = 0; ch < 3; ++ch) store_nt(s5, ch * 128 + 32 * d + i, v5[ch]);
        }
        if (d == 0 && lane == 0) {
#pragma unroll
            for (int ch = 0; ch < 3; ++ch) store_nt(s5, 3 * 128 + ch, t5[ch]);
        }
    }
}

template <bool W>
__global__ __launch_bounds__(kF2Threads, 1) void k_mlp_bwd3(int64_t m, const float *__restrict__ img, Bwd3Src src,
                                                            DwGrid g, float *__restrict__ slabs, InterpFuse ip,
                                                            const int *__restrict__ m_dev) {
    if (m_dev) m = __builtin_amdgcn_readfirstlane(*m_dev);
    mlp_bwd3_body<W>(blockIdx.x, gridDim.x, blockIdx.x, m, img, src, g, slabs, ip);
}

struct TrunkSrc {
    const int *m_dev;
    const float *g_sdf, *feat, *h2;
    const int *h2_src;
};
template <bool W, bool H2>
__global__ __launch_bounds__(kF2Threads, 1) void k_mlp_bwd3(int64_t m, const float *__restrict__ img, Bwd3Src src,
                                                            DwGrid g, float *__restrict__ slabs, InterpFuse ip,
                                                            const int *__restrict__ m_dev, TrunkSrc tk,
                                                            InterpFuse ip_b, BwdSplitCost cost) {
    static_assert(W, "the two-class launch is a training launch");
    const int n_wg = gridDim.x, b = blockIdx.x;
    if (m_dev) m = __builtin_amdgcn_readfirstlane(*m_dev);
    const int64_t m_b = __builtin_amdgcn_readfirstlane(*tk.m_dev);
    const int n_a = bwd_split_na((m + kU - 1) / kU, (m_b + kU - 1) / kU, n_wg, cost);
    if (b < n_a)
        mlp_bwd3_body<true>(b, n_a, b, m, img, src, g, slabs, ip);
    else
        mlp_trunk_fb_body<H2>(b - n_a, n_wg - n_a, b, m_b, img, tk.g_sdf, tk.feat, g, slabs, ip_b, tk.h2, tk.h2_src);
}

int bwd3_grid(int64_t m) {
    const int64_t rounds = (m + 4 * kU - 1) / (4 * kU);
    return persistent_grid(rounds > 0 ? rounds : 1);
}
constexpr int kDwRows[5] = {128, 128, 129, 128, 3};
constexpr int kDwCols[5] = {16, 128, 128, 144, 128};
void dw_grid_uniform(int n, DwGrid *g, int *slab_floats) {
    int off = 0;
    for (int l = 0; l < 5; ++l) {
        g->n_split[l] = n;
        g->slab_off[l] = off;
        g->slab_len[l] = kDwRows[l] * kDwCols[l] + kDwRows[l];
        off += n * g->slab_len[l];
    }
    *slab_floats = off;
}

}

int64_t dec128_workspace_floats(int64_t m) {
    DwGrid g;
    int slab;
    dw_grid_uniform(bwd3_grid(m), &g, &slab);
    return m * 3 + 2 * (int64_t)slab;
}

int dec128_bwd(hipStream_t st, int64_t m, const float *feat, const float *images, const float *rgb, const float *act,
               const uint64_t *masks, const float *g_sdf, const float *g_rgb, float *dfeat, float *const gw[5],
               float *const gb[5], int accumulate, int n_split, float *workspace, hipEvent_t dfeat_ready,
               const InterpFuse *ip, hipStream_t reduce_stream, const int *m_dev, const TrunkBwd *tb,
               const int *x_src) {
    PSVO_REQUIRE(m >= 0 && n_split > 0, "mlp_bwd: bad sizes");
    PSVO_REQUIRE(images != nullptr, "mlp_bwd: images of the training forward required");
    const bool want_w = gw[0] != nullptr;
    PSVO_REQUIRE(!want_w || act != nullptr, "mlp_bwd: weight gradients need the forward's activations");
    DwGrid g;
    int slab_floats;
    PSVO_REQUIRE(tb == nullptr || (gw[0] != nullptr && tb->m_dev && tb->g_sdf && tb->feat),
                 "mlp_bwd: the trunk backward needs the weight-gradient path and its inputs");
    float *slabs_b = nullptr;
    const int *cnt_a = nullptr, *cnt_b = nullptr;
    const BwdSplitCost cost = bwd_split_cost();
    auto reduce = [&](float *slabs, hipStream_t rs) {
        DwDst d;
        int e = 0;
        for (int l = 0; l < 5; ++l) {
            d.w[l] = gw[l];
            d.b[l] = gb[l];
            d.rows[l] = kDwRows[l];
            d.cols[l] = kDwCols[l];
            d.elem_begin[l] = e;
            e += kDwRows[l] * kDwCols[l] + kDwRows[l];
        }
        d.elem_begin[5] = e;
        psvo::launch(k_mlp_dw_reduce, dim3(div_up(e, kDwRedEl)), dim3(256), 0, rs, g, slabs, d, accumulate,
                     static_cast<const float *>(slabs_b), cnt_a, cnt_b, cost);
        return check_launch("mlp_dw_reduce");
    };
    Bwd3Src src{rgb, g_sdf, g_rgb, feat, masks, act, dfeat, x_src};
    if (!want_w) {
        if (m > 0) {
            launch_lds<k_mlp_bwd3<false>>(dim3(persistent_grid(div_up(div_up(m, kU), 8))), dim3(kF2Threads), kLdsBwd3,
                                          st, m, images, src, g, nullptr, InterpFuse{}, m_dev);
            const int rc = check_launch("mlp_bwd3");
            if (rc) return rc;
        }
        if (dfeat_ready && hipEventRecord(dfeat_ready, st) != hipSuccess)
            return set_error(PSVO_E_LAUNCH, "mlp_bwd: event record failed");
        return PSVO_OK;
    }
    const int grid = bwd3_grid(m);
    dw_grid_uniform(grid, &g, &slab_floats);
    float *slabs = workspace + m * 3;
    static const bool bind_env = [] {
        const char *v = getenv("PSVO_BIND_DFEAT");
        return !(v && v[0] == '0');
    }();
    const bool trunk_last = tb && m > 0;
    bool bound = false;
    const hipEvent_t bind_ev = bind_env ? dfeat_ready : nullptr;
    const bool one_launch = trunk_last && grid >= 2 && m_dev && !tb->two_launch;
    if (one_launch) {
        PSVO_REQUIRE(!tb->h2 || tb->src, "mlp_bwd: the trunk's h2 rows need their source index");
        cnt_a = m_dev;
        cnt_b = tb->m_dev;
        const TrunkSrc tk{tb->m_dev, tb->g_sdf, tb->feat, tb->h2, tb->src};
        const InterpFuse ip_a = ip ? *ip : InterpFuse{}, ip_b = tb->ip ? *tb->ip : InterpFuse{};
        constexpr int kLdsAb = kLdsBwd3 > kLdsTrunk ? kLdsBwd3 : kLdsTrunk;
        psvo::StopBind sb(bind_ev);
        if (tb->h2)
            launch_lds<k_mlp_bwd3<true, true>>(dim3(grid), dim3(kF2Threads), kLdsAb, st, m, images, src, g, slabs,
                                               ip_a, m_dev, tk, ip_b, cost);
        else
            launch_lds<k_mlp_bwd3<true, false>>(dim3(grid), dim3(kF2Threads), kLdsAb, st, m, images, src, g, slabs,
                                                ip_a, m_dev, tk, ip_b, cost);
        bound = sb.consumed();
        const int rc = check_launch("mlp_bwd3 (both classes)");
        if (rc) return rc;
    } else if (m > 0) {
        psvo::StopBind sb(trunk_last ? nullptr : bind_ev);
        launch_lds<k_mlp_bwd3<true>>(dim3(grid), dim3(kF2Threads), kLdsBwd3, st, m, images, src, g, slabs,
                                     ip ? *ip : InterpFuse{}, m_dev);
        bound = sb.consumed();
        const int rc = check_launch("mlp_bwd3");
        if (rc) return rc;
    } else if (hipMemsetAsync(slabs, 0, (size_t)slab_floats * sizeof(float), st) != hipSuccess) {
        return set_error(PSVO_E_LAUNCH, "mlp_bwd: memset failed");
    }
    if (trunk_last && !one_launch) {
        slabs_b = slabs + slab_floats;
        PSVO_REQUIRE(!tb->h2 || tb->src, "mlp_bwd: the trunk's h2 rows need their source index");
        psvo::StopBind sb(bind_ev);
        launch_trunk_fb(st, grid, images, *tb, g, slabs_b);
        bound = sb.consumed();
        const int rc = check_launch("mlp_trunk_fb");
        if (rc) return rc;
    }
    if (dfeat_ready && !bound && hipEventRecord(dfeat_ready, st) != hipSuccess)
        return set_error(PSVO_E_LAUNCH, "mlp_bwd: event record failed");
    if (reduce_stream && reduce_stream != st) {
        PSVO_REQUIRE(dfeat_ready != nullptr, "mlp_bwd: a separate reduce stream needs the dfeat_ready event");
        if (hipStreamWaitEvent(reduce_stream, dfeat_ready, 0) != hipSuccess)
            return set_error(PSVO_E_LAUNCH, "mlp_bwd: stream wait failed");
        return reduce(slabs, reduce_stream);
    }
    return reduce(slabs, st);
}

}
```

### proud-slam_amd/csrc/psvo_common.h

```cpp
#pragma once

#include <hip/hip_ext.h>
#include <hip/hip_runtime.h>
#include <stdint.h>

#include "../../include/psvo.h"

namespace psvo {

struct KernelClock {
    static constexpr int kMax = 192, kMaxInst = 64;
    hipEvent_t ev[kMax][2] = {};
    int region[kMax] = {};
    int n = 0;
    struct Inst {
        int region, first, last;
    } inst[kMaxInst] = {};
    int n_inst = 0;
    int stack[8] = {};
    int depth = 0;
    bool sum = false;
    bool overflow = false;
    hipStream_t streams[4] = {};
    bool owns(hipStream_t st) const {
// ... 173 lines not shown
int64_t dec256_tiles16(int64_t m);
int64_t dec256_image_floats();
int64_t dec256_act_floats(int64_t m);
int64_t dec256_mask_words(int64_t m);
int64_t dec256_workspace_floats(int64_t m);
int dec256_images(hipStream_t st, const float *const *dec, float *images);
int dec256_fwd(hipStream_t st, int64_t m, const float *feat, const float *const *dec, float *images, float *sdf,
               float *rgb, float *act, uint64_t *masks, const int *m_dev = nullptr);
struct InterpFuse;
int dec256_bwd(hipStream_t st, int64_t m, const float *feat, const float *images, const float *rgb, const float *act,
               const uint64_t *masks, const float *g_sdf, const float *g_rgb, float *dfeat, float *const gw[5],
               float *const gb[5], int accumulate, float *workspace, hipEvent_t dfeat_ready,
               const InterpFuse *ip = nullptr, const int *m_dev = nullptr);

struct H2Rows;
struct TrunkBwd;
int64_t dec128_image_floats();
int64_t dec128_act_floats(int64_t m);
int64_t dec128_mask_words(int64_t m);
int64_t dec128_workspace_floats(int64_t m);
int dec128_images(hipStream_t st, const float *const *dec, float *images);
int dec128_fwd(hipStream_t st, int64_t m, const float *feat, const float *const *dec, float *images, float *sdf,
               float *rgb, float *act, uint64_t *masks, const int *m_dev, const H2Rows *h2);
int dec128_bwd(hipStream_t st, int64_t m, const float *feat, const float *images, const float *rgb, const float *act,
               const uint64_t *masks, const float *g_sdf, const float *g_rgb, float *dfeat, float *const gw[5],
               float *const gb[5], int accumulate, int n_split, float *workspace, hipEvent_t dfeat_ready,
               const InterpFuse *ip, hipStream_t reduce_stream, const int *m_dev, const TrunkBwd *tb,
               const int *x_src);

constexpr int kXchMaxFrames = 64;

struct RenderWs;
RenderWs *&engine_render_ws(psvo_engine *e);
bool engine_data_parallel(const psvo_engine *e);
void render_ws_free(RenderWs *ws);

typedef __attribute__((address_space(1))) int g_i32;
typedef __attribute__((address_space(1))) float g_f32;
typedef __attribute__((address_space(1))) unsigned long long g_u64;
__device__ __forceinline__ void st_wt(int *p, int v) {
    __hip_atomic_store((g_i32 *)p, v, __ATOMIC_RELAXED, __HIP_MEMORY_SCOPE_AGENT);
}
__device__ __forceinline__ void st_wt(float *p, float v) {
    __hip_atomic_store((g_f32 *)p, v, __ATOMIC_RELAXED, __HIP_MEMORY_SCOPE_AGENT);
}
__device__ __forceinline__ int ld_wt(const int *p) {
    return __hip_atomic_load((g_i32 *)p, __ATOMIC_RELAXED, __HIP_MEMORY_SCOPE_AGENT);
}
__device__ __forceinline__ float ld_wt(const float *p) {
    return __hip_atomic_load((g_f32 *)p, __ATOMIC_RELAXED, __HIP_MEMORY_SCOPE_AGENT);
}
__device__ __forceinline__ void stat_to_host(unsigned long long *host, int word, int v, int seq) {
    __hip_atomic_store((g_u64 *)(host + word), ((unsigned long long)(unsigned)seq << 32) | (unsigned)v,
                       __ATOMIC_RELAXED, __HIP_MEMORY_SCOPE_SYSTEM);
}
__device__ __forceinline__ void crit_coef_from_counts(double n_valid_d, double n_f_d, double n_s_d, double n_hit,
                                                      double n_cols, float rgb_w, float depth_w, float fs_w,
                                                      float sdf_w, float tr, int flags, float *coef) {
    const double n_el = n_hit * n_cols;
    const float n_valid = (float)n_valid_d;
    const float n_f = (float)n_f_d, n_s = (float)n_s_d;
    const float n_tot = n_s + n_f;
    const float fs_weight = 1.0f - n_f / n_tot;
    const float sdf_weight = 1.0f - n_s / n_tot;
    coef[0] = (flags & PSVO_CRIT_USE_COLOR) ? (float)(rgb_w / (3.0 * n_hit)) : 0.0f;
    coef[1] = (flags & PSVO_CRIT_USE_DEPTH) ? depth_w / n_valid : 0.0f;
    coef[2] = (flags & PSVO_CRIT_USE_SDF) ? (float)(2.0 * (double)(fs_w * fs_weight) / n_el) : 0.0f;
    coef[3] = (flags & PSVO_CRIT_USE_SDF) ? (float)(2.0 * (double)(sdf_w * sdf_weight) / n_el) * tr : 0.0f;
}

struct InterpFuse {
    const int *leaf, *ray_of, *rank_ray, *vertex_idx;
    const float *t, *rays_o, *rays_d, *centres, *emb;
    float voxel_size;
    float *grad_emb;
    float *gx;
    uint8_t *row_flags;
};

int interp_rays_gx(hipStream_t st, int64_t r_hit, const int *offsets, const int *ray_index, const float *t,
                   const float *gx, float *grad_o, float *grad_d, const int *offsets2 = nullptr,
                   const float *t2 = nullptr, const float *gx2 = nullptr);

struct TrunkBwd {
    const int *m_dev;
    const float *g_sdf, *feat;
    const InterpFuse *ip;
    const float *h2 = nullptr;
    const int *src = nullptr;
    bool two_launch = false;
};

struct BwdSplitCost {
    int a, b, b0;
};
constexpr BwdSplitCost kBwdSplitCost = {75, 35, 16};
BwdSplitCost bwd_split_cost();
__host__ __device__ inline int64_t bwd_split_rounds(int64_t units, int n) { return ((units + n - 1) / n + 3) / 4; }
__host__ __device__ inline int bwd_split_na(int64_t units_a, int64_t units_b, int n_wg, BwdSplitCost c) {
    if (units_a <= 0) return 0;
    if (units_b <= 0 || n_wg < 2) return n_wg;
    auto t_a = [&](int n) { return bwd_split_rounds(units_a, n) * c.a; };
    auto t_b = [&](int n) { return bwd_split_rounds(units_b, n_wg - n) * c.b + c.b0; };
    int lo = 1, hi = n_wg - 1;
    while (lo < hi) {
        const int mid = (lo + hi) / 2;
        if (t_a(mid) <= t_b(mid))
            hi = mid;
        else
            lo = mid + 1;
    }
    auto t = [&](int n) {
        const int64_t ta = t_a(n), tb = t_b(n);
        return ta > tb ? ta : tb;
    };
    return lo > 1 && t(lo - 1) < t(lo) ? lo - 1 : lo;
}
int mlp_bwd(void *stream, int64_t m, int width, const float *feat, const float *images, const float *rgb,
            const float *act, const uint64_t *masks, const float *g_sdf, const float *g_rgb, float *dfeat,
            float *const *grads, int accumulate, int n_split, float *workspace, hipEvent_t dfeat_ready,
            const InterpFuse *ip = nullptr, hipStream_t reduce_stream = nullptr, const int *m_dev = nullptr,
            const TrunkBwd *tb = nullptr,
            const int *x_src = nullptr);
bool mlp_bwd_fuses_interp(int width);
bool mlp_bwd_split_tail(int width);

int mlp_images(void *stream, int width, const float *const *dec, float *images);
struct H2Rows {
    float *out = nullptr;
    const float *rows = nullptr;
    const int *src = nullptr;
};
int mlp_fwd_prepared(void *stream, int64_t m, int width, const float *feat, float *images, float *sdf, float *rgb,
                     float *act, uint64_t *masks, const int *m_dev = nullptr,
                     const H2Rows *h2 = nullptr);
int mlp_fwd(void *stream, int64_t m, int width, const float *feat, const float *const *dec, float *images, float *sdf,
            float *rgb, float *act, uint64_t *masks);

}

#define PSVO_REQUIRE(cond, ...)                                       \
    do {                                                              \
        if (!(cond)) return ::psvo::set_error(PSVO_E_INVALID, __VA_ARGS__); \
    } while (0)
```

### proud-slam_amd/psvo/_lib.py

```python
from __future__ import annotations

import ctypes
import os

import torch

PKG_ROOT = os.path.dirname(os.path.dirname(os.path.abspath(__file__)))
LIB_PATH = os.environ.get("PSVO_LIB_PATH") or os.path.join(PKG_ROOT, "lib", "libpsvo.so")

_vp, _i32, _i64, _f32, _f64, _u64 = (ctypes.c_void_p, ctypes.c_int, ctypes.c_int64, ctypes.c_float,
                                      ctypes.c_double, ctypes.c_uint64)

_SIGNATURES = {
    "psvo_last_error": (ctypes.c_char_p, []),
    "psvo_version": (ctypes.c_char_p, []),
    "psvo_svo_intersect": (_i32, [_vp, _i32, _i32, _i32, _f32, _i32] + [_vp] * 7),
    "psvo_inverse_cdf_sampling": (_i32, [_vp, _i32, _i32, _i32, _i32, _f32] + [_vp] * 9),
    "psvo_ball_intersect": (_i32, [_vp, _i32, _i32, _i32, _f32, _i32] + [_vp] * 6),
    "psvo_aabb_intersect": (_i32, [_vp, _i32, _i32, _i32, _f32, _i32] + [_vp] * 6),
    "psvo_triangle_intersect": (_i32, [_vp, _i32, _i32, _i32, _f32, _f32, _i32] + [_vp] * 6),
    "psvo_uniform_ray_sampling": (_i32, [_vp, _i32, _i32, _i32, _i32, _f32] + [_vp] * 7),
    "psvo_ray_intersect_sorted": (_i32, [_vp, _i64, _vp, _vp, _vp, _vp, _f32, _f32, _f32] + [_vp] * 6),
    "psvo_hit_rank": (_i32, [_vp, _i64, _vp, _vp, _vp]),
    "psvo_sample_rays": (_i32, [_vp, _i64, _i32, _vp, _vp, _vp, _vp, _vp, _f32, _vp, _u64, _vp, _vp, _vp, _vp,
                                _vp, _vp]),
    "psvo_sample_rays_range": (_i32, [_vp, _i64, _i64, _i64, _i32, _vp, _vp, _vp, _vp, _vp, _f32, _vp, _u64, _vp,
                                      _vp, _vp, _vp, _vp, _vp]),
    "psvo_ray_stats": (_i32, [_vp, _i64, _vp, _vp, _f32, _vp]),
    "psvo_scan_counts": (_i32, [_vp, _i64, _vp, _vp]),
    "psvo_sample_points": (_i32, [_vp, _i64, _i32, _i32] + [_vp] * 9),
    "psvo_interp_fwd": (_i32, [_vp, _i64, _i32, _f32] + [_vp] * 9),
    "psvo_interp_bwd": (_i32, [_vp, _i64, _i32, _f32] + [_vp] * 12),
    "psvo_interp_bwd_workspace_floats": (_i64, [_i64, _i32]),
    "psvo_interp_bwd_chunked": (_i32, [_vp, _i64, _i32, _i32, _f32] + [_vp] * 13),
    "psvo_composite_fwd": (_i32, [_vp, _i64, _i32, _f32] + [_vp] * 10),
    "psvo_composite_bwd": (_i32, [_vp, _i64, _i32, _f32] + [_vp] * 12),
    "psvo_composite_loss": (_i32, [_vp, _i64, _i32, _f32, _f32] + [_vp] * 14),
    "psvo_criterion_coef": (_i32, [_vp, _i64, _i32, _f32, _f32, _vp, _vp, _vp, _f32, _f32, _f32, _f32, _i32, _vp,
                                   _vp, _vp]),
    "psvo_criterion_reduce": (_i32, [_vp, _i64, _vp, _vp]),
    "psvo_rows_workspace_ints": (_i64, [_i64]),
    "psvo_sample_pixels_workspace_ints": (_i64, [_i32, _i64]),
    "psvo_pack_tree_workspace_ints": (_i64, [_i64]),
    "psvo_adam_mark_rows": (_i32, [_vp, _i64, _vp, _vp, _vp]),
    "psvo_adam_flags_from_state": (_i32, [_vp, _i64, _vp, _vp, _vp]),
    "psvo_pack_tree": (_i32, [_vp, _i64, _vp, _vp, _vp, _vp]),
    "psvo_ray_intersect_sorted_packed": (_i32, [_vp, _i64, _vp, _vp, _vp, _vp, _vp, _f32, _f32, _f32] + [_vp] * 6),
    "psvo_sample_pixels": (_i32, [_vp, _i32, _i64, _i64, _vp, _i32, _vp, _u64, _vp, _vp, _vp, _vp, _vp, _vp]),
    "psvo_rows_compact": (_i32, [_vp, _i64, _i32, _vp, _vp, _vp, _vp, _vp]),
    "psvo_rows_scatter_add": (_i32, [_vp, _i64, _i32, _vp, _vp, _vp]),
    "psvo_rows_compact_flagged": (_i32, [_vp, _i64, _i32, _vp, _vp, _vp, _vp, _vp, _vp]),
    "psvo_rows_clear": (_i32, [_vp, _i64, _i32, _vp, _vp, _vp]),
    "psvo_rows_mark": (_i32, [_vp, _i64, _vp, _vp]),
    "psvo_rows_flags_from_grad": (_i32, [_vp, _i64, _i32, _vp, _vp]),
    "psvo_mlp_image_floats": (_i64, []),
    "psvo_mlp_image_floats_w": (_i64, [_i32]),
    "psvo_mlp_act_floats": (_i64, [_i64, _i32]),
    "psvo_mlp_mask_words": (_i64, [_i64, _i32]),
    "psvo_mlp_workspace_floats_w": (_i64, [_i64, _i32, _i32]),
    "psvo_map_grad_floats_w": (_i64, [_i64, _i32]),
    "psvo_mlp_fwd": (_i32, [_vp, _i64, _i32] + [_vp] * 16),
    "psvo_mlp_workspace_floats": (_i64, [_i64, _i32]),
    "psvo_mlp_bwd": (_i32, [_vp, _i64, _i32] + [_vp] * 28 + [_i32, _i32, _vp]),
    "psvo_criterion_workspace_floats": (_i64, [_i64]),
    "psvo_criterion_sums": (_i32, [_vp, _i64, _i32, _i32, _f32, _f32] + [_vp] * 9),
    "psvo_criterion_finalize": (_i32, [_vp, _vp, _i64, _i32, _f32, _f32, _f32, _f32, _f32, _i32, _vp]),
    "psvo_criterion_bwd": (_i32, [_vp, _i64, _i32, _f32, _f32] + [_vp] * 12),
    "psvo_adam_step": (_i32, [_vp, _i32, _vp, _vp, _vp, _vp, _vp, _f64, _f64, _f64, _f64, _f64, _i64]),
    "psvo_engine_new": (_vp, []),
    "psvo_engine_free": (None, [_vp]),
    "psvo_engine_set_timing": (_i32, [_vp, _i32]),
    "psvo_engine_set_paths": (_i32, [_vp, _i32]),
    "psvo_engine_select_stats": (_i32, [_vp, _vp, _vp, _i32]),
    "psvo_engine_gate_stream": (_i32, [_vp, _vp]),
    "psvo_debug_set_lookback": (_i32, [_i32, _i32, _i32]),
    "psvo_debug_set_bwd_split": (_i32, [_i32, _i32, _i32]),
    "psvo_debug_bwd_split": (_i32, [_i64, _i64, _i32]),
    "psvo_debug_set_pixel_draw": (_i32, [_i32]),
    "psvo_debug_lb_helps": (_i32, [_vp, _i32]),
    "psvo_debug_select_samples": (_i32, [_vp, _i64, _i32, _f32, _f32, _vp, _vp, _vp, _i32] + [_vp] * 7
                                  + [_i64, _i32] + [_vp] * 11 + [ctypes.c_uint32, _vp]),
    "psvo_debug_select_granules": (_i64, [_i64]),
    "psvo_debug_trunk_interp": (_i32, [_vp, _i32, _i64] + [_vp] * 10 + [_f32] + [_vp] * 14),
    "psvo_debug_composite_loss": (_i32, [_vp, _i64, _i32, _f32, _f32, _vp, _vp, _vp, _i32] + [_vp] * 11
                                  + [_i32, _vp]),
    "psvo_engine_queued": (_i32, [_vp]),
    "psvo_map_discard": (_i32, [_vp]),
    "psvo_engine_exchange_words": (_i64, [_i32, _i64, _i64]),
    "psvo_engine_set_exchange": (_i32, [_vp, _i32, _i32, _i64, _i64, _vp, _vp, _vp, _vp]),
    "psvo_engine_timing": (_i32, [_vp, _vp]),
    "psvo_engine_set_clock": (_i32, [_vp, _i32]),
    "psvo_engine_clock": (_i32, [_vp, _vp, _vp]),
    "psvo_host_wait_stats": (_i32, [_vp, _vp, _vp, _i32]),
    "psvo_map_step": (_i32, [_vp, _vp, _vp, _i64, _vp, _vp, _vp, _vp, _u64, _i64, _i32, _vp, _vp]),
    "psvo_map_adam": (_i32, [_vp, _vp, _vp, _i64]),
    "psvo_map_adam_ex": (_i32, [_vp, _vp, _vp, _i64, _i32]),
    "psvo_map_join": (_i32, [_vp, _vp]),
    "psvo_map_side_wait": (_i32, [_vp, _vp]),
    "psvo_engine_grad_rays": (_i32, [_vp, _vp, _i64, _vp, _vp]),
    "psvo_map_query": (_i32, [_vp, _vp, _vp, _i64, _vp, _vp, _u64]),
    "psvo_map_step_frames": (_i32, [_vp, _vp, _vp, _vp, _vp, _vp, _vp, _u64, _i64, _i32, _vp, _vp]),
    "psvo_pose_rays_frames": (_i32, [_vp, _i64, _i64, _vp, _vp, _vp, _vp]),
    "psvo_pose_grad_frames": (_i32, [_vp, _i32, _i64, _i64, _vp, _vp, _vp, _vp, _vp, _vp]),
    "psvo_track_step": (_i32, [_vp, _vp, _vp, _i64, _vp, _vp, _vp, _vp, _vp, _vp, _f64, _vp, _u64, _i64, _i32, _vp,
                               _vp, _vp]),
    "psvo_render_frame": (_i32, [_vp, _vp, _vp, _i64, _vp, _vp, _vp, _u64, _vp, _vp, _vp, _vp, _vp, _vp]),
    "psvo_render_tile_bytes": (_i64, [_i64, _i32, _i32]),
    "psvo_pose_rays": (_i32, [_vp, _i64, _vp, _vp, _vp, _vp]),
    "psvo_mesh_linspace": (_i32, [_i32, _vp]),
    "psvo_mesh_case_table": (_i32, [_vp, _vp]),
    "psvo_mesh_grid_feat": (_i32, [_vp, _i64, _i32, _f32, _vp, _vp, _vp, _vp]),
    "psvo_mesh_point_feat": (_i32, [_vp, _i64, _f32, _vp, _vp, _vp, _vp, _vp, _vp]),
    "psvo_mesh_mc_count": (_i32, [_vp, _i64, _i32] + [_vp] * 6),
    "psvo_mesh_mc_emit": (_i32, [_vp, _i64, _i32, _f32] + [_vp] * 7),
    "psvo_mesh_vox_map_slots": (_i64, [_i64]),
    "psvo_mesh_vertex_rows": (_i32, [_vp, _i64, _vp, _i64, _vp, _f32, _vp, _vp]),
    "psvo_mesh_depth_points": (_i32, [_vp, _i64, _vp, _vp, _vp, _vp]),
    "psvo_mesh_downsample_workspace_bytes": (_i64, [_i64]),
    "psvo_mesh_points_downsample": (_i32, [_vp, _i64, _vp, _f64, _vp, _vp, _vp]),
    "psvo_mesh_points_status": (_i32, [_i64]),
    "psvo_mesh_ball_workspace_bytes": (_i64, [_i64]),
    "psvo_mesh_ball_any": (_i32, [_vp, _i64, _vp, _i64, _vp, _f64, _vp, _vp, _vp]),
    "psvo_pose_grad": (_i32, [_vp, _i64, _vp, _vp, _vp, _vp, _vp, _vp]),
    "psvo_criterion_depth_filter": (_i32, [_vp, _i64, _i32] + [_vp] * 7),
    "psvo_criterion_sums_ex": (_i32, [_vp, _i64, _i32, _i32, _f32, _f32] + [_vp] * 11),
    "psvo_criterion_bwd_ex": (_i32, [_vp, _i64, _i32, _f32, _f32] + [_vp] * 14),
    "psvo_map_grad_floats": (_i64, [_i64]),
    "psvo_dtree_new": (_vp, [_vp, _i32, _i64]),
    "psvo_dtree_free": (None, [_vp]),
    "psvo_dtree_insert": (_i32, [_vp, _vp, _vp, _i64]),
    "psvo_dtree_count": (_i64, [_vp]),
    "psvo_dtree_count_leaves": (_i64, [_vp, _vp]),
    "psvo_dtree_export": (_i32, [_vp, _vp, _f32, _vp, _vp, _vp, _vp, _vp]),
    "psvo_dtree_probe": (_i32, [_vp, _vp, _vp, _i64, _i32, _vp]),
    "psvo_dtree_generation": (_u64, [_vp]),
    "psvo_depth_voxel_keys": (_i32, [_vp, _i64, _vp, _vp, _vp, _f32, _vp, _vp]),
    "psvo_dtree_frame_workspace_bytes": (_i64, [_i32, _i32]),
    "psvo_dtree_insert_depth": (_i32, [_vp, _vp, _i32, _i32, _vp, _vp, _vp, _f32, _vp]),
    "psvo_share_block_bytes": (_i64, []),
    "psvo_share_create": (_vp, [ctypes.c_char_p]),
    "psvo_share_attach": (_vp, [ctypes.c_char_p]),
    "psvo_share_detach": (None, [_vp]),
    "psvo_share_unlink": (_i32, [ctypes.c_char_p]),
    "psvo_share_set_flag": (_i32, [_vp, _i32, _i32]),
    "psvo_share_get_flag": (_i32, [_vp, _i32]),
    "psvo_share_push_pose": (_i32, [_vp, _vp, _i32]),
    "psvo_share_trajectory": (_i64, [_vp, _vp, _i64]),
    "psvo_share_publish": (_i32, [_vp, _vp, _i32, _i32, _vp, _vp, _vp, _i64, _i32, _vp, _vp]),
    "psvo_share_acquire": (_i32, [_vp, _i32, _u64, _vp, _vp, _vp, _i64, _vp, _vp, _vp]),
    "psvo_share_read": (_i32, [_vp, _vp, _i32, _i32, _i32, _vp, _vp, _vp, _vp]),
    "psvo_share_release": (_i32, [_vp, _i32, _i32]),
    "psvo_share_version": (_u64, [_vp, _i32]),
    "psvo_octree_new": (_vp, [_i32, _i32, _f64, _i32]),
    "psvo_octree_free": (None, [_vp]),
    "psvo_octree_insert": (_i32, [_vp, _vp, _i64]),
# ... 83 lines not shown
```

### proud-slam_amd/psvo/engine.py

```python
from __future__ import annotations

import ctypes
import os

import torch

from . import _lib as L

_vp, _i32, _i64, _f32, _f64 = ctypes.c_void_p, ctypes.c_int, ctypes.c_int64, ctypes.c_float, ctypes.c_double


class MapDesc(ctypes.Structure):
    _fields_ = [("n_nodes", _i64), ("centres", _vp), ("structure", _vp), ("vertex_idx", _vp),
                ("emb", _vp), ("n_emb", _i64), ("emb_m", _vp), ("emb_v", _vp),
                ("dec", _vp * 10), ("dec_m", _vp * 10), ("dec_v", _vp * 10), ("width", _i32),
                ("voxel_size", _f32), ("step_size", _f32), ("max_distance", _f32), ("truncation", _f32),
                ("max_depth", _f32), ("w_rgb", _f32), ("w_depth", _f32), ("w_fs", _f32), ("w_sdf", _f32),
                ("lr_emb", _f64), ("lr_dec", _f64), ("beta1", _f64), ("beta2", _f64), ("eps", _f64),
                ("grad_flat", _vp), ("packed", _vp), ("emb_row_flags", _vp), ("emb_row_local", _vp)]


class MapFrames(ctypes.Structure):
    _fields_ = [("n_frames", _i32), ("rays_per_frame", _i64), ("dirs_cam", _vp), ("poses", _vp), ("pose_m", _vp),
                ("pose_v", _vp), ("pose_step", _vp), ("lr_pose", _f64), ("pose_grad", _vp),
# ... 194 lines not shown
        rd = torch.empty_like(dirs)
        L.call("psvo_pose_rays_frames", L.stream_of(dirs.device), dirs.shape[0], rpf, poses, dirs, ro, rd)
        d = self.desc
        q = _intersect_sorted(ro, rd, self.centres, self.structure, d.voxel_size, d.max_distance, d.step_size)
        st = q["stats"].cpu()
        P, r_hit, max_ceil = int(st[0]), int(st[1]), int(st[2])
        want = (200, (r_hit + 199) // 200, max_ceil + P)
        if tuple(nz.shape) != want:
            raise ValueError(f"step_frames: noise must be {list(want)} for this batch, got {list(nz.shape)}")

    def set_exchange(self, exchange):
        n = int(_lib().psvo_engine_exchange_words(exchange.world, exchange.max_rays_global, exchange.max_rays_rank))
        if n < 0:
            raise ValueError(f"EngineExchange: bad sizes (max_rays_global {exchange.max_rays_global}, "
                             f"max_rays_rank {exchange.max_rays_rank})")
        xi32, xf64 = exchange.buffers(n)
        if xi32.device != self.emb.device:
            raise RuntimeError("EngineExchange buffers must live on the engine's device")
        L.call("psvo_engine_set_exchange", self.handle, exchange.rank, exchange.world, exchange.max_rays_global,
               exchange.max_rays_rank, ctypes.cast(exchange.callback(), _vp), None, xi32, xf64)
        self.exchange = exchange
        if self.row_flags is not None and self.row_local is None:
            self.row_local = torch.zeros_like(self.row_flags)
            self.desc.emb_row_local = self.row_local.data_ptr()
        from .dist import EngineGradExchange
        self.grad_exchange = EngineGradExchange(self, op="sum", group=exchange.group,
                                                force=getattr(exchange, "force", False))

    def _error(self, name, rc):
        msg = _lib().psvo_last_error().decode()
        if self.exchange is not None and self.exchange.error is not None:
            msg += f" ({type(self.exchange.error).__name__}: {self.exchange.error})"
            self.exchange.error = None
        return L.PsvoError(f"{name} failed (code {rc}): {msg}")

    def discard_queued(self):
        L.call("psvo_map_discard", self.handle)
        self._queued.clear()
        self._ahead = None

    def _sync_queue(self):
        n = int(_lib().psvo_engine_queued(self.handle))
        while len(self._queued) > n:
            self._queued.pop(0)

    def query(self, rays_o, rays_d, seed):
        ro = rays_o.reshape(-1, 3).float().contiguous()
        rd = rays_d.reshape(-1, 3).float().contiguous()
        rc = _lib().psvo_map_query(self.handle, L.stream_of(ro.device), ctypes.addressof(self.desc), ro.shape[0],
                                   ro.data_ptr(), rd.data_ptr(), int(seed))
        if rc != 0:
            raise self._error("psvo_map_query", rc)
        self._queued.append((rays_o, rays_d, int(seed), ro, rd))

    def step(self, rays_o, rays_d, rgb, depth, seed, apply_adam=True):
        if self._queued:
            q_o, q_d, q_seed, ro, rd = self._queued[0]
            if q_o is not rays_o or q_d is not rays_d or q_seed != int(seed):
                raise RuntimeError("MappingEngine.step: rays / seed differ from the batch query() queued "
                                   "(pass the same tensor objects and seed)")
        else:
            ro = rays_o.reshape(-1, 3).float().contiguous()
            rd = rays_d.reshape(-1, 3).float().contiguous()
        gt_rgb = rgb.reshape(-1, 3).float().contiguous()
        gt_d = depth.reshape(-1).float().contiguous()
        self.step_no += 1
        rc = _lib().psvo_map_step(self.handle, L.stream_of(ro.device), ctypes.addressof(self.desc), ro.shape[0],
                                  ro.data_ptr(), rd.data_ptr(), gt_rgb.data_ptr(), gt_d.data_ptr(), int(seed),
                                  self.step_no, 0 if apply_adam else 1, self.loss_out.data_ptr(),
                                  ctypes.addressof(self.stats))
        self._sync_queue()
        if rc != 0:
            self.step_no -= 1
            raise self._error("psvo_map_step", rc)
        return self.loss_out[0]

    def adam(self):
        ge = self.grad_exchange
        marked = ge is not None and ge.take_rows_marked()
        L.call("psvo_map_adam_ex", self.handle, L.stream_of(self.emb.device), ctypes.addressof(self.desc),
               self.step_no, 1 if marked else 0)

    PATH_QUERY_SPLIT, PATH_PADDED, PATH_DENSE_DECODER, PATH_INTERP_PASS, PATH_BWD_TWO_LAUNCH = 1, 2, 4, 8, 16

    def set_paths(self, paths):
        L.call("psvo_engine_set_paths", self.handle, int(paths))

    def select_stats(self, reset=False):
        out = (ctypes.c_int64 * 5)()
        L.call("psvo_engine_select_stats", self.handle, L.stream_of(self.emb.device), ctypes.cast(out, ctypes.c_void_p),
               int(bool(reset)))
        return {"kept": out[0], "composited": out[1], "kept_sum": out[2], "composited_sum": out[3], "steps": out[4]}

    def set_timing(self, on):
        L.call("psvo_engine_set_timing", self.handle, 2 if on == "overlap" else int(bool(on)))

    def set_clock(self, max_steps):
        L.call("psvo_engine_set_clock", self.handle, int(max_steps))

    def clock(self):
        ms, n = ctypes.c_double(), ctypes.c_int()
        L.call("psvo_engine_clock", self.handle, ctypes.byref(ms), ctypes.byref(n))
        return (ms.value if ms.value >= 0 else None), n.value

    @staticmethod
    def host_wait_stats(reset=False):
        us, calls, waited = ctypes.c_double(), ctypes.c_longlong(), ctypes.c_longlong()
        L.call("psvo_host_wait_stats", ctypes.byref(us), ctypes.byref(calls), ctypes.byref(waited), int(reset))
        return us.value, calls.value, waited.value

    REGIONS = ("mlp_fwd", "mlp_bwd", "interp_fwd", "interp_bwd", "intersect", "sample", "points", "select")

    def timing(self):
        out = (ctypes.c_double * len(self.REGIONS))()
        L.call("psvo_engine_timing", self.handle, ctypes.cast(out, ctypes.c_void_p))
        return dict(zip(self.REGIONS, list(out)))

    @property
    def last_stats(self):
        return list(self.stats)

    def close(self):
        if getattr(self, "handle", None) is not None:
            _lib().psvo_engine_free(self.handle)
            self.handle = None

    def __del__(self):
        try:
            self.close()
        except Exception:
            pass


class TrackingEngine:

    def __init__(self, map_states, decoder, voxel_size, step_size, truncation=0.1, max_distance=10.0,
                 criteria=None, max_depth=10.0, betas=(0.9, 0.999), eps=1e-8):
        crit = criteria or {"rgb_weight": 0.5, "depth_weight": 1.0, "sdf_weight": 5000.0, "fs_weight": 10.0}
        emb = map_states["voxel_vertex_emb"].detach()
        self.params = [p.detach() for p in decoder.fused_params()]
        for t in [emb] + self.params:
            if not (t.is_cuda and t.dtype == torch.float32 and t.is_contiguous()):
                raise RuntimeError("TrackingEngine: embeddings / decoder parameters must be contiguous f32 CUDA")
        self.dev = emb.device
        self.emb = emb
        self.centres = map_states["voxel_center_xyz"].float().contiguous()
        self.structure = map_states["voxel_structure"].int().contiguous()
        self.vertex_idx = map_states["voxel_vertex_idx"].int().contiguous()
        d = MapDesc()
        d.n_nodes = self.centres.shape[0]
        d.centres, d.structure, d.vertex_idx = (t.data_ptr() for t in (self.centres, self.structure,
                                                                        self.vertex_idx))
        d.emb, d.n_emb = emb.data_ptr(), emb.shape[0]
        for i in range(10):
            d.dec[i] = self.params[i].data_ptr()
        d.width = decoder.W
        d.voxel_size, d.step_size, d.max_distance, d.truncation = voxel_size, step_size, max_distance, truncation
        d.max_depth = max_depth
        d.w_rgb, d.w_depth = crit["rgb_weight"], crit["depth_weight"]
        d.w_fs, d.w_sdf = crit["fs_weight"], crit["sdf_weight"]
        d.beta1, d.beta2, d.eps = betas[0], betas[1], eps
        self.desc = d
        self.pose = torch.zeros(6, dtype=torch.float32, device=self.dev)
        self.pose_m = torch.zeros(6, dtype=torch.float32, device=self.dev)
        self.pose_v = torch.zeros(6, dtype=torch.float32, device=self.dev)
        self.pose_grad = torch.zeros(8, dtype=torch.float32, device=self.dev)
        self.loss_out = torch.empty(16, dtype=torch.float32, device=self.dev)
        self.stats = (ctypes.c_int * 16)()
        self.step_no = 0
# ... 61 lines not shown
```

Measured before the change: 6.546 million.

## Fuse composite loss pass into one-launch MLP backward kernel prologue

Moves the per-ray composite loss and gradient computation out of its own kernel and into a prologue of the one-launch two-class MLP backward kernel. Each workgroup first computes the loss gradients for its own row range, with a separate sample-wise path for the trunk class. A new PATH_LOSS_PASS flag keeps the separate pass available. Wave reductions also switch to permlane swaps and DPP moves instead of shuffles. This removes a kernel launch and a round trip of gradients through memory, at the cost of extra register and latency pressure in the large backward kernel, and redundant work at the boundaries of the ray ranges.

```diff
diff --git a/include/psvo.h b/include/psvo.h
--- a/include/psvo.h
+++ b/include/psvo.h
@@ -286,9 +286,11 @@
     PSVO_PATH_PADDED = 2,
     PSVO_PATH_DENSE_DECODER = 4,
     PSVO_PATH_INTERP_PASS = 8,
-    PSVO_PATH_BWD_TWO_LAUNCH = 16
+    PSVO_PATH_BWD_TWO_LAUNCH = 16,
+    PSVO_PATH_LOSS_PASS = 32
 };
 int psvo_engine_set_paths(psvo_engine *e, int paths);
+int psvo_engine_loss_in_bwd(psvo_engine *e);
 
 int psvo_engine_select_stats(psvo_engine *e, void *stream, int64_t *out, int reset);
 
diff --git a/proud-slam_amd/csrc/composite.hip b/proud-slam_amd/csrc/composite.hip
--- a/proud-slam_amd/csrc/composite.hip
+++ b/proud-slam_amd/csrc/composite.hip
@@ -1,5 +1,6 @@
 #include <hip/hip_runtime.h>
 
+#include "composite_ray.h"
 #include "lookback.h"
 #include "psvo_common.h"
 #include "query.h"
@@ -7,38 +8,6 @@
 
 namespace psvo {
 namespace {
-
-__device__ __forceinline__ float wsum(float v) {
-#pragma unroll
-    for (int s = 32; s > 0; s >>= 1) v += __shfl_xor(v, s, 64);
-    return v;
-}
-__device__ __forceinline__ int wmin(int v) {
-#pragma unroll
-    for (int s = 32; s > 0; s >>= 1) v = min(v, __shfl_xor(v, s, 64));
-    return v;
-}
-__device__ __forceinline__ float sigm(float x) { return 1.0f / (1.0f + expf(-x)); }
-
-__device__ __forceinline__ float comp_gw3(float gdp, float z, float gwx, bool has_c, float c0, float c1, float c2,
-                                          float gr, float gg, float gb) {
-    const float g = fmaf(gdp, z, gwx);
-    return has_c ? fmaf(gb, c2, fmaf(gg, c1, fmaf(gr, c0, g))) : g;
-}
-__device__ __forceinline__ float comp_gw(float gdp, float z, float gwx, const float *c, float gr, float gg, float gb) {
-    return c ? comp_gw3(gdp, z, gwx, true, c[0], c[1], c[2], gr, gg, gb) : comp_gw3(gdp, z, gwx, false, 0.f, 0.f,
-                                                                                   0.f, gr, gg, gb);
-}
-__device__ __forceinline__ float comp_gsdf_sig(float gw, float dot, float tot, bool keep, float sp, float sn, float tr,
-                                               float g) {
-    const float gu = keep ? (gw - dot) / tot : 0.f;
-    const float du = sp * sn * (sn - sp) / tr;
-    return fmaf(gu, du, g);
-}
-__device__ __forceinline__ float comp_gsdf(float gw, float dot, float tot, bool keep, float sdf, float tr, float g) {
-    const float a = sdf / tr;
-    return comp_gsdf_sig(gw, dot, tot, keep, sigm(a), sigm(-a), tr, g);
-}
 
 __global__ __launch_bounds__(256) void k_composite_fwd(int64_t r_hit, int s_max, float tr,
                                                        const int *__restrict__ offsets,
@@ -157,31 +126,6 @@
     }
 }
 
-constexpr int kPartColor = 0, kPartDepth = 1, kPartQFs = 5, kPartQSdf = 6, kPartN = 8;
-
-struct CritTerms {
-    float f, sm, xfs, ysdf;
-};
-__device__ __forceinline__ CritTerms crit_terms(float z, float p, float d, float tr, float max_depth) {
-#pragma clang fp contract(off)
-    CritTerms o;
-    o.f = z < (d - tr) ? 1.0f : 0.0f;
-    const float b = z > (d + tr) ? 1.0f : 0.0f;
-    const float dm = (d > 0.0f && d < max_depth) ? 1.0f : 0.0f;
-    o.sm = (1.0f - o.f) * (1.0f - b) * dm;
-    o.xfs = p * o.f - o.f;
-    o.ysdf = (z + p * tr) * o.sm - d * o.sm;
-    return o;
-}
-__device__ __forceinline__ float crit_sq_add(float acc, float x) {
-#pragma clang fp contract(off)
-    return acc + x * x;
-}
-__device__ __forceinline__ float crit_grad(float cfs, float csdf, const CritTerms &t) {
-#pragma clang fp contract(off)
-    return cfs * t.xfs * t.f + csdf * t.ysdf * t.sm;
-}
-
 template <int J>
 __global__ __launch_bounds__(256) void k_composite_loss(int64_t r_hit, int s_max, float tr, float max_depth,
                                                         const int *__restrict__ offsets,
@@ -199,174 +143,10 @@
     const int lane = threadIdx.x & 63;
     const int64_t r = (int64_t)blockIdx.x * (blockDim.x >> 6) + (threadIdx.x >> 6);
     if (r >= r_hit) return;
-    const int64_t orig = rank_ray[r];
-    const int off = offsets[r], ns = ray_ns[r];
-    const int lim = ns < s_max ? ns : s_max;
-    const float d = gt_depth[orig];
-    const float gt0 = gt_rgb[orig * 3 + 0], gt1 = gt_rgb[orig * 3 + 1], gt2 = gt_rgb[orig * 3 + 2];
-    const float ccol = coef[0], cdep = coef[1], cfs = coef[2], csdf = coef[3];
-    const float *z = z_vals + r * z_stride;
-    auto z_at = [&](int s) { return s < ns ? z[s] : kMaxDepthFill; };
-    auto sdf_at = [&](int s) { return s < ns ? sdf_s[off + s] : 1.0f; };
-    auto ci_at = [&](int s) { return s < ns ? (cidx ? cidx[off + s] : off + s) : -1; };
-    constexpr int JR = J > 0 ? J : 1;
-    float zr[JR], pr[JR], c0r[JR], c1r[JR], c2r[JR];
-    if constexpr (J > 0) {
-#pragma unroll
-        for (int j = 0; j < J; ++j) {
-            const int s = lane + 64 * j;
-            zr[j] = s < s_max ? z_at(s) : 0.f;
-            pr[j] = sdf_at(s);
-            const int ci = ci_at(s);
-            const bool v = ci >= 0;
-            const float *c = rgb_s + (int64_t)(v ? ci : 0) * 3;
-            c0r[j] = v ? c[0] : 0.f;
-            c1r[j] = v ? c[1] : 0.f;
-            c2r[j] = v ? c[2] : 0.f;
-        }
-    }
-    auto Z = [&](int j, int s) {
-        if constexpr (J > 0) return zr[j]; else return z_at(s);
-    };
-    auto P = [&](int j, int s) {
-        if constexpr (J > 0) return pr[j]; else return sdf_at(s);
-    };
-    auto C = [&](int j, int s, int k) {
-        if constexpr (J > 0) return k == 0 ? c0r[j] : (k == 1 ? c1r[j] : c2r[j]);
-        else {
-            const int ci = ci_at(s);
-            return ci >= 0 ? rgb_s[(int64_t)ci * 3 + k] : 0.f;
-        }
-    };
-#define PSVO_FOR_S(lim) for (int j = 0, s = lane; (J == 0 || j < J) && s < (lim); ++j, s += 64)
-    float pn[JR];
-    if constexpr (J > 0) {
-#pragma unroll
-        for (int j = 0; j < J; ++j) {
-            const float dn = __shfl_down(pr[j], 1, 64);
-            const float nx = __shfl(pr[j + 1 < J ? j + 1 : j], 0, 64);
-            pn[j] = lane < 63 ? dn : nx;
-        }
-    }
-    int first = s_max;
-    PSVO_FOR_S(lim) {
-        const float v = P(j, s);
-        float v1;
-        if constexpr (J > 0) v1 = pn[j];
-        else v1 = s + 1 < s_max ? sdf_at(s + 1) : 0.f;
-        if (s + 1 < s_max && v1 * v < 0.0f) first = min(first, s);
-    }
-    first = wmin(first);
-    const float zmin = z_at(first == s_max ? 0 : first);
-    float spr[JR], snr[JR], wr[JR];
-#pragma unroll
-    for (int j = 0; j < JR; ++j) spr[j] = snr[j] = wr[j] = 0.f;
-    float tot = 0.f;
-    PSVO_FOR_S(lim) {
-        const float a = P(j, s) / tr;
-        const float sp = sigm(a), sn = sigm(-a);
-        float w = sp * sn;
-        const bool keep = (Z(j, s) < zmin + tr) && (s < ns);
-        tot += keep ? w : 0.0f;
-        if constexpr (J > 0) {
-            spr[j] = sp;
-            snr[j] = sn;
-            wr[j] = keep ? w : 0.0f;
-        }
-    }
-    tot = wsum(tot) + 1e-8f;
-    if constexpr (J > 0) {
-#pragma unroll
-        for (int j = 0; j < J; ++j) wr[j] = wr[j] / tot;
-    }
-    auto weight_at = [&](int j, int s) {
-        if constexpr (J > 0) {
-            return wr[j];
-        } else {
-            const float a = P(j, s) / tr;
-            const float w = sigm(a) * sigm(-a);
-            const bool keep = (Z(j, s) < zmin + tr) && (s < ns);
-            return (keep ? w : 0.0f) / tot;
-        }
-    };
-    float cr = 0.f, cg = 0.f, cb = 0.f, dd = 0.f;
-    PSVO_FOR_S(lim) {
-        const float w = weight_at(j, s);
-        if (s < ns) {
-            cr += w * C(j, s, 0);
-            cg += w * C(j, s, 1);
-            cb += w * C(j, s, 2);
-        }
-        dd += w * Z(j, s);
-    }
-    cr = wsum(cr);
-    cg = wsum(cg);
-    cb = wsum(cb);
-    dd = wsum(dd);
-    float qfs = 0.f, qsdf = 0.f;
-    if (partials) {
-        PSVO_FOR_S(s_max) {
-            const CritTerms t = crit_terms(Z(j, s), P(j, s), d, tr, max_depth);
-            qfs = crit_sq_add(qfs, t.xfs);
-            qsdf = crit_sq_add(qsdf, t.ysdf);
-        }
-        qfs = wsum(qfs);
-        qsdf = wsum(qsdf);
-    }
-    const float rgb[3] = {cr, cg, cb};
-    const float gt[3] = {gt0, gt1, gt2};
-    float gcol[3], ac = 0.f;
-#pragma unroll
-    for (int c = 0; c < 3; ++c) {
-        const float e = gt[c] - rgb[c];
-        ac += fabsf(e);
-        gcol[c] = -ccol * (e > 0.0f ? 1.0f : (e < 0.0f ? -1.0f : 0.0f));
-    }
-    const bool valid = d > 0.01f && d < max_depth;
-    const float ed = d - dd;
-    const float gdp = valid ? -cdep * (ed > 0.0f ? 1.0f : (ed < 0.0f ? -1.0f : 0.0f)) : 0.0f;
-    if (lane == 0) {
-        color[r * 3 + 0] = cr;
-        color[r * 3 + 1] = cg;
-        color[r * 3 + 2] = cb;
-        depth[r] = dd;
-        if (partials) {
-            float *o = part + r * kPartN;
-            o[kPartColor] = ac;
-            o[kPartDepth] = valid ? fabsf(ed) : 0.0f;
-            o[kPartQFs] = qfs;
-            o[kPartQSdf] = qsdf;
-            o[7] = 0.0f;
-        }
-    }
-    float dot = 0.f;
-    PSVO_FOR_S(lim) {
-        const bool v = s < ns;
-        const float gw = comp_gw3(gdp, Z(j, s), 0.f, v, v ? C(j, s, 0) : 0.f, v ? C(j, s, 1) : 0.f,
-                                  v ? C(j, s, 2) : 0.f, gcol[0], gcol[1], gcol[2]);
-        dot = fmaf(gw, weight_at(j, s), dot);
-    }
-    dot = wsum(dot);
-    PSVO_FOR_S(ns) {
-        const float W = weight_at(j, s);
-        const float zs = Z(j, s);
-        const float gw = comp_gw3(gdp, zs, 0.f, true, C(j, s, 0), C(j, s, 1), C(j, s, 2), gcol[0], gcol[1], gcol[2]);
-        const float p = P(j, s);
-        const float gsdf = crit_grad(cfs, csdf, crit_terms(zs, p, d, tr, max_depth));
-        const int gi = ci_at(s);
-        if (gi < 0) continue;
-        if constexpr (J > 0)
-            g_sdf_s[gi] = comp_gsdf_sig(gw, dot, tot, zs < zmin + tr, spr[j], snr[j], tr, gsdf);
-        else
-            g_sdf_s[gi] = comp_gsdf(gw, dot, tot, zs < zmin + tr, p, tr, gsdf);
-        float *gc = g_rgb_s + (int64_t)gi * 3;
-        gc[0] = W * gcol[0];
-        gc[1] = W * gcol[1];
-        gc[2] = W * gcol[2];
-    }
-#undef PSVO_FOR_S
-}
-
+    composite_loss_ray<J, false>(r, lane, s_max, tr, max_depth, offsets, ray_ns, z_vals, z_stride, rank_ray, gt_rgb,
+                                 gt_depth, sdf_s, rgb_s, coef, part, color, depth, g_sdf_s, g_rgb_s, partials, cidx,
+                                 RayRows{0, 0, true});
+}
 
 constexpr int kSelWaves = 8, kSelMaxRpw = 16;
 struct SelectArgs {
@@ -642,10 +422,9 @@
                      workspace && color && depth && grad_sdf_s && grad_rgb_s,
                  "composite_loss: null pointer");
     if (r_hit == 0) return PSVO_OK;
-    auto kern = s_max <= 128   ? k_composite_loss<2>
-                : s_max <= 256 ? k_composite_loss<4>
-                : s_max <= 512 ? k_composite_loss<8>
-                               : k_composite_loss<0>;
+    const int J = composite_loss_j(s_max);
+    auto kern = J == 2 ? k_composite_loss<2> : J == 4 ? k_composite_loss<4> : J == 8 ? k_composite_loss<8>
+                                                                                      : k_composite_loss<0>;
     psvo::launch(kern, dim3(div_up(r_hit, 4)), dim3(256), 0, as_stream(stream), r_hit, s_max, truncation,
                        max_depth, offsets, ray_ns, z_vals, z_stride, rank_ray, gt_rgb, gt_depth, sdf_s, rgb_s, coef,
                        workspace, color, depth, grad_sdf_s, grad_rgb_s, partials ? 1 : 0, cidx);
diff --git a/proud-slam_amd/csrc/composite_ray.h b/proud-slam_amd/csrc/composite_ray.h
--- /dev/null
+++ b/proud-slam_amd/csrc/composite_ray.h
@@ -0,0 +1,361 @@
+#pragma once
+#ifndef PSVO_HOST_SHIM
+#include <hip/hip_runtime.h>
+
+#include "psvo_common.h"
+#endif
+
+namespace psvo {
+namespace {
+
+#ifdef PSVO_HOST_SHIM
+__device__ __forceinline__ float wsum(float v) {
+    for (int s = 32; s > 0; s >>= 1) v += __shfl_xor(v, s, 64);
+    return v;
+}
+__device__ __forceinline__ int wmin(int v) {
+    for (int s = 32; s > 0; s >>= 1) v = min(v, __shfl_xor(v, s, 64));
+    return v;
+}
+#else
+template <int CTRL>
+__device__ __forceinline__ int lane_dpp(int x) {
+    return __builtin_amdgcn_mov_dpp(x, CTRL, 0xF, 0xF, false);
+}
+constexpr int kDppRor8 = 0x128, kDppRor4 = 0x124, kDppXor2 = 0x4E, kDppXor1 = 0xB1;
+__device__ __forceinline__ float wsum(float v) {
+    auto h = __builtin_amdgcn_permlane32_swap(__float_as_uint(v), __float_as_uint(v), false, false);
+    v = __uint_as_float(h[0]) + __uint_as_float(h[1]);
+    h = __builtin_amdgcn_permlane16_swap(__float_as_uint(v), __float_as_uint(v), false, false);
+    v = __uint_as_float(h[0]) + __uint_as_float(h[1]);
+    v += __int_as_float(lane_dpp<kDppRor8>(__float_as_int(v)));
+    v += __int_as_float(lane_dpp<kDppRor4>(__float_as_int(v)));
+    v += __int_as_float(lane_dpp<kDppXor2>(__float_as_int(v)));
+    v += __int_as_float(lane_dpp<kDppXor1>(__float_as_int(v)));
+    return v;
+}
+__device__ __forceinline__ int wmin(int v) {
+    auto h = __builtin_amdgcn_permlane32_swap((unsigned)v, (unsigned)v, false, false);
+    v = min((int)h[0], (int)h[1]);
+    h = __builtin_amdgcn_permlane16_swap((unsigned)v, (unsigned)v, false, false);
+    v = min((int)h[0], (int)h[1]);
+    v = min(v, lane_dpp<kDppRor8>(v));
+    v = min(v, lane_dpp<kDppRor4>(v));
+    v = min(v, lane_dpp<kDppXor2>(v));
+    v = min(v, lane_dpp<kDppXor1>(v));
+    return v;
+}
+#endif
+__device__ __forceinline__ float sigm(float x) { return 1.0f / (1.0f + expf(-x)); }
+
+__device__ __forceinline__ float comp_gw3(float gdp, float z, float gwx, bool has_c, float c0, float c1, float c2,
+                                          float gr, float gg, float gb) {
+    const float g = fmaf(gdp, z, gwx);
+    return has_c ? fmaf(gb, c2, fmaf(gg, c1, fmaf(gr, c0, g))) : g;
+}
+__device__ __forceinline__ float comp_gw(float gdp, float z, float gwx, const float *c, float gr, float gg, float gb) {
+    return c ? comp_gw3(gdp, z, gwx, true, c[0], c[1], c[2], gr, gg, gb) : comp_gw3(gdp, z, gwx, false, 0.f, 0.f,
+                                                                                   0.f, gr, gg, gb);
+}
+__device__ __forceinline__ float comp_gsdf_sig(float gw, float dot, float tot, bool keep, float sp, float sn, float tr,
+                                               float g) {
+    const float gu = keep ? (gw - dot) / tot : 0.f;
+    const float du = sp * sn * (sn - sp) / tr;
+    return fmaf(gu, du, g);
+}
+__device__ __forceinline__ float comp_gsdf(float gw, float dot, float tot, bool keep, float sdf, float tr, float g) {
+    const float a = sdf / tr;
+    return comp_gsdf_sig(gw, dot, tot, keep, sigm(a), sigm(-a), tr, g);
+}
+
+constexpr int kPartColor = 0, kPartDepth = 1, kPartQFs = 5, kPartQSdf = 6, kPartN = 8;
+
+struct CritTerms {
+    float f, sm, xfs, ysdf;
+};
+__device__ __forceinline__ CritTerms crit_terms(float z, float p, float d, float tr, float max_depth) {
+#pragma clang fp contract(off)
+    CritTerms o;
+    o.f = z < (d - tr) ? 1.0f : 0.0f;
+    const float b = z > (d + tr) ? 1.0f : 0.0f;
+    const float dm = (d > 0.0f && d < max_depth) ? 1.0f : 0.0f;
+    o.sm = (1.0f - o.f) * (1.0f - b) * dm;
+    o.xfs = p * o.f - o.f;
+    o.ysdf = (z + p * tr) * o.sm - d * o.sm;
+    return o;
+}
+__device__ __forceinline__ float crit_sq_add(float acc, float x) {
+#pragma clang fp contract(off)
+    return acc + x * x;
+}
+__device__ __forceinline__ float crit_grad(float cfs, float csdf, const CritTerms &t) {
+#pragma clang fp contract(off)
+    return cfs * t.xfs * t.f + csdf * t.ysdf * t.sm;
+}
+
+struct RayRows {
+    int64_t lo, hi;
+    bool owner;
+};
+
+__host__ __device__ constexpr int composite_loss_j(int s_max) {
+    return s_max <= 128 ? 2 : s_max <= 256 ? 4 : s_max <= 512 ? 8 : 0;
+}
+
+template <int J, bool Filter, int NB>
+__device__ __forceinline__ void composite_loss_rays(const int64_t (&r)[NB], const int lane, int s_max, float tr,
+                                                    float max_depth, const int *offsets, const int *ray_ns,
+                                                    const float *z_vals, int z_stride, const int *rank_ray,
+                                                    const float *gt_rgb, const float *gt_depth, const float *sdf_s,
+                                                    const float *rgb_s, const float *coef, float *part, float *color,
+                                                    float *depth, float *g_sdf_s, float *g_rgb_s, int partials,
+                                                    const int *cidx, const RayRows (&rows)[NB]) {
+#define PSVO_FOR_B _Pragma("unroll") for (int b = 0; b < NB; ++b)
+    int64_t orig[NB];
+    int off[NB], ns[NB];
+    PSVO_FOR_B {
+        orig[b] = rank_ray[r[b]];
+        off[b] = offsets[r[b]];
+        ns[b] = ray_ns[r[b]];
+    }
+    int lim[NB];
+    float d[NB], gt0[NB], gt1[NB], gt2[NB];
+    const float *z[NB];
+    PSVO_FOR_B {
+        lim[b] = ns[b] < s_max ? ns[b] : s_max;
+        d[b] = gt_depth[orig[b]];
+        gt0[b] = gt_rgb[orig[b] * 3 + 0];
+        gt1[b] = gt_rgb[orig[b] * 3 + 1];
+        gt2[b] = gt_rgb[orig[b] * 3 + 2];
+        z[b] = z_vals + r[b] * z_stride;
+    }
+    const float ccol = coef[0], cdep = coef[1], cfs = coef[2], csdf = coef[3];
+    auto z_at = [&](int b, int s) { return s < ns[b] ? z[b][s] : kMaxDepthFill; };
+    auto sdf_at = [&](int b, int s) { return s < ns[b] ? sdf_s[off[b] + s] : 1.0f; };
+    auto ci_at = [&](int b, int s) { return s < ns[b] ? (cidx ? cidx[off[b] + s] : off[b] + s) : -1; };
+    constexpr int JR = J > 0 ? J : 1;
+    float zr[NB][JR], pr[NB][JR], c0r[NB][JR], c1r[NB][JR], c2r[NB][JR];
+    if constexpr (J > 0) {
+        int cir[NB][JR];
+        PSVO_FOR_B {
+#pragma unroll
+            for (int j = 0; j < J; ++j) {
+                const int s = lane + 64 * j;
+                zr[b][j] = s < s_max ? z_at(b, s) : 0.f;
+                pr[b][j] = sdf_at(b, s);
+                cir[b][j] = ci_at(b, s);
+            }
+        }
+        PSVO_FOR_B {
+#pragma unroll
+            for (int j = 0; j < J; ++j) {
+                const int ci = cir[b][j];
+                const bool v = ci >= 0;
+                const float *c = rgb_s + (int64_t)(v ? ci : 0) * 3;
+                c0r[b][j] = v ? c[0] : 0.f;
+                c1r[b][j] = v ? c[1] : 0.f;
+                c2r[b][j] = v ? c[2] : 0.f;
+            }
+        }
+    }
+    auto Z = [&](int b, int j, int s) {
+        if constexpr (J > 0) return zr[b][j]; else return z_at(b, s);
+    };
+    auto P = [&](int b, int j, int s) {
+        if constexpr (J > 0) return pr[b][j]; else return sdf_at(b, s);
+    };
+    auto C = [&](int b, int j, int s, int k) {
+        if constexpr (J > 0) return k == 0 ? c0r[b][j] : (k == 1 ? c1r[b][j] : c2r[b][j]);
+        else {
+            const int ci = ci_at(b, s);
+            return ci >= 0 ? rgb_s[(int64_t)ci * 3 + k] : 0.f;
+        }
+    };
+#define PSVO_FOR_S(lim) for (int j = 0, s = lane; (J == 0 || j < J) && s < (lim); ++j, s += 64)
+    float pn[NB][JR];
+    if constexpr (J > 0) {
+        PSVO_FOR_B {
+#pragma unroll
+            for (int j = 0; j < J; ++j) {
+                const float dn = __shfl_down(pr[b][j], 1, 64);
+                const float nx = __shfl(pr[b][j + 1 < J ? j + 1 : j], 0, 64);
+                pn[b][j] = lane < 63 ? dn : nx;
+            }
+        }
+    }
+    int first[NB];
+    PSVO_FOR_B {
+        first[b] = s_max;
+        PSVO_FOR_S(lim[b]) {
+            const float v = P(b, j, s);
+            float v1;
+            if constexpr (J > 0) v1 = pn[b][j];
+            else v1 = s + 1 < s_max ? sdf_at(b, s + 1) : 0.f;
+            if (s + 1 < s_max && v1 * v < 0.0f) first[b] = min(first[b], s);
+        }
+    }
+    PSVO_FOR_B first[b] = wmin(first[b]);
+    float zmin[NB];
+    PSVO_FOR_B {
+        const int f = first[b] == s_max ? 0 : first[b];
+        if constexpr (J > 0) {
+            float zs = zr[b][0];
+#pragma unroll
+            for (int j = 1; j < J; ++j) zs = (f >> 6) == j ? zr[b][j] : zs;
+            zmin[b] = __shfl(zs, f & 63, 64);
+        } else {
+            zmin[b] = z_at(b, f);
+        }
+    }
+    float spr[NB][JR], snr[NB][JR], wr[NB][JR];
+    float tot[NB];
+    PSVO_FOR_B {
+#pragma unroll
+        for (int j = 0; j < JR; ++j) spr[b][j] = snr[b][j] = wr[b][j] = 0.f;
+        tot[b] = 0.f;
+        PSVO_FOR_S(lim[b]) {
+            const float a = P(b, j, s) / tr;
+            const float sp = sigm(a), sn = sigm(-a);
+            float w = sp * sn;
+            const bool keep = (Z(b, j, s) < zmin[b] + tr) && (s < ns[b]);
+            tot[b] += keep ? w : 0.0f;
+            if constexpr (J > 0) {
+                spr[b][j] = sp;
+                snr[b][j] = sn;
+                wr[b][j] = keep ? w : 0.0f;
+            }
+        }
+    }
+    PSVO_FOR_B tot[b] = wsum(tot[b]) + 1e-8f;
+    if constexpr (J > 0) {
+        PSVO_FOR_B {
+#pragma unroll
+            for (int j = 0; j < J; ++j) wr[b][j] = wr[b][j] / tot[b];
+        }
+    }
+    auto weight_at = [&](int b, int j, int s) {
+        if constexpr (J > 0) {
+            return wr[b][j];
+        } else {
+            const float a = P(b, j, s) / tr;
+            const float w = sigm(a) * sigm(-a);
+            const bool keep = (Z(b, j, s) < zmin[b] + tr) && (s < ns[b]);
+            return (keep ? w : 0.0f) / tot[b];
+        }
+    };
+    float cr[NB], cg[NB], cb[NB], dd[NB];
+    PSVO_FOR_B {
+        cr[b] = cg[b] = cb[b] = dd[b] = 0.f;
+        PSVO_FOR_S(lim[b]) {
+            const float w = weight_at(b, j, s);
+            if (s < ns[b]) {
+                cr[b] += w * C(b, j, s, 0);
+                cg[b] += w * C(b, j, s, 1);
+                cb[b] += w * C(b, j, s, 2);
+            }
+            dd[b] += w * Z(b, j, s);
+        }
+    }
+    PSVO_FOR_B {
+        cr[b] = wsum(cr[b]);
+        cg[b] = wsum(cg[b]);
+        cb[b] = wsum(cb[b]);
+        dd[b] = wsum(dd[b]);
+    }
+    float qfs[NB], qsdf[NB];
+    PSVO_FOR_B qfs[b] = qsdf[b] = 0.f;
+    if (partials) {
+        PSVO_FOR_B {
+            PSVO_FOR_S(s_max) {
+                const CritTerms t = crit_terms(Z(b, j, s), P(b, j, s), d[b], tr, max_depth);
+                qfs[b] = crit_sq_add(qfs[b], t.xfs);
+                qsdf[b] = crit_sq_add(qsdf[b], t.ysdf);
+            }
+            qfs[b] = wsum(qfs[b]);
+            qsdf[b] = wsum(qsdf[b]);
+        }
+    }
+    float gcol[NB][3], gdp[NB];
+    PSVO_FOR_B {
+        const float rgb[3] = {cr[b], cg[b], cb[b]};
+        const float gt[3] = {gt0[b], gt1[b], gt2[b]};
+        float ac = 0.f;
+#pragma unroll
+        for (int c = 0; c < 3; ++c) {
+            const float e = gt[c] - rgb[c];
+            ac += fabsf(e);
+            gcol[b][c] = -ccol * (e > 0.0f ? 1.0f : (e < 0.0f ? -1.0f : 0.0f));
+        }
+        const bool valid = d[b] > 0.01f && d[b] < max_depth;
+        const float ed = d[b] - dd[b];
+        gdp[b] = valid ? -cdep * (ed > 0.0f ? 1.0f : (ed < 0.0f ? -1.0f : 0.0f)) : 0.0f;
+        if (lane == 0 && (!Filter || rows[b].owner)) {
+            color[r[b] * 3 + 0] = cr[b];
+            color[r[b] * 3 + 1] = cg[b];
+            color[r[b] * 3 + 2] = cb[b];
+            depth[r[b]] = dd[b];
+            if (partials) {
+                float *o = part + r[b] * kPartN;
+                o[kPartColor] = ac;
+                o[kPartDepth] = valid ? fabsf(ed) : 0.0f;
+                o[kPartQFs] = qfs[b];
+                o[kPartQSdf] = qsdf[b];
+                o[7] = 0.0f;
+            }
+        }
+    }
+    float dot[NB];
+    PSVO_FOR_B {
+        dot[b] = 0.f;
+        PSVO_FOR_S(lim[b]) {
+            const bool v = s < ns[b];
+            const float gw = comp_gw3(gdp[b], Z(b, j, s), 0.f, v, v ? C(b, j, s, 0) : 0.f, v ? C(b, j, s, 1) : 0.f,
+                                      v ? C(b, j, s, 2) : 0.f, gcol[b][0], gcol[b][1], gcol[b][2]);
+            dot[b] = fmaf(gw, weight_at(b, j, s), dot[b]);
+        }
+    }
+    PSVO_FOR_B dot[b] = wsum(dot[b]);
+    PSVO_FOR_B {
+        PSVO_FOR_S(ns[b]) {
+            const float W = weight_at(b, j, s);
+            const float zs = Z(b, j, s);
+            const float gw = comp_gw3(gdp[b], zs, 0.f, true, C(b, j, s, 0), C(b, j, s, 1), C(b, j, s, 2), gcol[b][0],
+                                      gcol[b][1], gcol[b][2]);
+            const float p = P(b, j, s);
+            const float gsdf = crit_grad(cfs, csdf, crit_terms(zs, p, d[b], tr, max_depth));
+            const int gi = ci_at(b, s);
+            if (gi < 0) continue;
+            if constexpr (Filter) {
+                if (gi < rows[b].lo || gi >= rows[b].hi) continue;
+            }
+            if constexpr (J > 0)
+                g_sdf_s[gi] = comp_gsdf_sig(gw, dot[b], tot[b], zs < zmin[b] + tr, spr[b][j], snr[b][j], tr, gsdf);
+            else
+                g_sdf_s[gi] = comp_gsdf(gw, dot[b], tot[b], zs < zmin[b] + tr, p, tr, gsdf);
+            float *gc = g_rgb_s + (int64_t)gi * 3;
+            gc[0] = W * gcol[b][0];
+            gc[1] = W * gcol[b][1];
+            gc[2] = W * gcol[b][2];
+        }
+    }
+#undef PSVO_FOR_S
+#undef PSVO_FOR_B
+}
+
+template <int J, bool Filter>
+__device__ __forceinline__ void composite_loss_ray(const int64_t r, const int lane, int s_max, float tr,
+                                                   float max_depth, const int *offsets, const int *ray_ns,
+                                                   const float *z_vals, int z_stride, const int *rank_ray,
+                                                   const float *gt_rgb, const float *gt_depth, const float *sdf_s,
+                                                   const float *rgb_s, const float *coef, float *part, float *color,
+                                                   float *depth, float *g_sdf_s, float *g_rgb_s, int partials,
+                                                   const int *cidx, const RayRows rows) {
+    const int64_t rr[1] = {r};
+    const RayRows rw[1] = {rows};
+    composite_loss_rays<J, Filter, 1>(rr, lane, s_max, tr, max_depth, offsets, ray_ns, z_vals, z_stride, rank_ray,
+                                      gt_rgb, gt_depth, sdf_s, rgb_s, coef, part, color, depth, g_sdf_s, g_rgb_s,
+                                      partials, cidx, rw);
+}
+
+}
+}
diff --git a/proud-slam_amd/csrc/engine.cpp b/proud-slam_amd/csrc/engine.cpp
--- a/proud-slam_amd/csrc/engine.cpp
+++ b/proud-slam_amd/csrc/engine.cpp
@@ -249,6 +249,8 @@
     if (ipass && ipass[0] == '1') e->paths |= PSVO_PATH_INTERP_PASS;
     const char *two = getenv("PSVO_BWD_TWO_LAUNCH");
     if (two && two[0] == '1') e->paths |= PSVO_PATH_BWD_TWO_LAUNCH;
+    const char *lpass = getenv("PSVO_LOSS_PASS");
+    if (lpass && lpass[0] == '1') e->paths |= PSVO_PATH_LOSS_PASS;
     for (auto &q : e->qs)
         if (query_set_init(q) != PSVO_OK) {
             psvo_engine_free(e);
@@ -291,9 +293,11 @@
     return PSVO_OK;
 }
 
+extern "C" int psvo_engine_loss_in_bwd(psvo_engine *e) { return e && e->loss_in_bwd ? 1 : 0; }
+
 extern "C" int psvo_engine_set_paths(psvo_engine *e, int paths) {
     PSVO_REQUIRE(e && (paths & ~(PSVO_PATH_QUERY_SPLIT | PSVO_PATH_PADDED | PSVO_PATH_DENSE_DECODER |
-                               PSVO_PATH_INTERP_PASS | PSVO_PATH_BWD_TWO_LAUNCH)) == 0,
+                               PSVO_PATH_INTERP_PASS | PSVO_PATH_BWD_TWO_LAUNCH | PSVO_PATH_LOSS_PASS)) == 0,
                  "engine_set_paths: bad arguments");
     PSVO_REQUIRE(e->q_count == 0, "engine_set_paths: queries are queued");
     e->paths = paths;
diff --git a/proud-slam_amd/csrc/engine_internal.h b/proud-slam_amd/csrc/engine_internal.h
--- a/proud-slam_amd/csrc/engine_internal.h
+++ b/proud-slam_amd/csrc/engine_internal.h
@@ -129,6 +129,7 @@
     bool images_next = false;
     const float *images_w0 = nullptr;
     int paths = 0;
+    bool loss_in_bwd = false;
     int64_t m_early = 0;
     uint32_t sel_tag = 0;
     uint32_t sel_zero_gen = 0;
diff --git a/proud-slam_amd/csrc/engine_step.cpp b/proud-slam_amd/csrc/engine_step.cpp
--- a/proud-slam_amd/csrc/engine_step.cpp
+++ b/proud-slam_amd/csrc/engine_step.cpp
@@ -408,6 +408,9 @@
     int *cidx = nullptr, *sel_cnt = nullptr, *offb = nullptr;
     const int *h2_src = nullptr;
     float *crit_ws = nullptr, *coef = nullptr, *g_sdf_s = nullptr, *g_rgb_s = nullptr;
+    bool coef_q = false;
+    bool loss_fused = false;
+    psvo::LossFuse lossf{};
     double *sums = nullptr;
     float *grads = nullptr, *grad_od = nullptr;
     float *G[10] = {};
@@ -516,6 +519,7 @@
     const bool coef_q = !s.dist && s.counts_gt && qset->counts_gt == s.counts_gt;
     const bool sums_q = s.dist && s.counts_gt && qset->counts_gt != nullptr &&
                         !(qset->host_stats[PSVO_STAT_FLAGS] & psvo::PSVO_FLAG_UNION_UNCOUNTED);
+    s.coef_q = coef_q;
     s.coef = coef_q ? static_cast<float *>(qset->a.p[kCoefQ]) : nullptr;
     if (!coef_q) {
         ENG_BUF(float, cbuf, kCoef, 4 * sizeof(float));
@@ -556,6 +560,17 @@
     ENG_BUF(float, g_rgb_s, kGRgbS, s.m_rows() * 3 * sizeof(float));
     s.g_sdf_s = g_sdf_s;
     s.g_rgb_s = g_rgb_s;
+    s.loss_fused = s.two_class() && !s.want_loss && !s.dist && s.coef_q && !s.empty && q.r_hit > 0 && s.h2_src &&
+                   !(e->paths & PSVO_PATH_LOSS_PASS) &&
+                   psvo::dec128_bwd_one_launch(q.m, s.sel_cnt != nullptr, (e->paths & PSVO_PATH_BWD_TWO_LAUNCH) != 0);
+    e->loss_in_bwd = s.loss_fused;
+    if (s.loss_fused) {
+        s.lossf = psvo::LossFuse{q.s_max,   q.z_stride, d->truncation, d->max_depth, q.s.offsets, q.ray_ns,
+                                 q.rank_ray, s.cidx,     s.k.ray_of,    s.h2_src,     q.z_vals,    s.gt_rgb,
+                                 s.gt_depth, q.sdf_s,    s.k.rgb_s,     s.coef,       g_sdf_s,     g_rgb_s,
+                                 q.m};
+        return PSVO_OK;
+    }
     if (!s.empty)
         ENG_CALL(psvo::composite_loss_z(st, q.r_hit, q.s_max, d->truncation, d->max_depth, q.s.offsets, q.ray_ns,
                                         q.z_vals, q.z_stride, q.rank_ray, s.gt_rgb, s.gt_depth, q.sdf_s, s.k.rgb_s,
@@ -639,7 +654,7 @@
                                  d->centres, d->emb, d->voxel_size, grad_emb, gx ? gx + 3 * M : nullptr, s.mark_into};
     const psvo::TrunkBwd tbw{s.sel_cnt ? s.sel_cnt + 1 : nullptr, s.g_sdf_s + M, s.h2_src ? k.feat : k.feat + M * 16,
                              fuse_ib ? &ipf_b : nullptr, s.h2_src ? q.h2 : nullptr, s.h2_src ? s.h2_src + M : nullptr,
-                             (e->paths & PSVO_PATH_BWD_TWO_LAUNCH) != 0};
+                             (e->paths & PSVO_PATH_BWD_TWO_LAUNCH) != 0, s.loss_fused ? &s.lossf : nullptr};
     ENG_CALL(mlp_bwd(st, M, d->width, k.feat, q.images, k.rgb_s, k.act, k.masks, s.g_sdf_s, s.g_rgb_s, dfeat, s.G, 0,
                      n_split, mlp_ws, s.overlap ? e->dfeat_ready : nullptr, fuse_ib ? &ipf : nullptr,
                      s.split ? ax : nullptr, s.sel_cnt, s.two_class() ? &tbw : nullptr, s.h2_src));
diff --git a/proud-slam_amd/csrc/mlp128.h b/proud-slam_amd/csrc/mlp128.h
--- a/proud-slam_amd/csrc/mlp128.h
+++ b/proud-slam_amd/csrc/mlp128.h
@@ -174,10 +174,19 @@
             psvo_g_stamps[kStampK][blockIdx.x][threadIdx.x >> 6][stit_][i] = t_;                         \
     } while (0)
 #define PSVO_STAMP_FLUSH(k) ++stit_
+#define PSVO_STAMP_AT(k, it, i)                                                                     \
+    do {                                                                                            \
+        __builtin_amdgcn_sched_barrier(0);                                                          \
+        const unsigned long long t_ = __builtin_amdgcn_s_memtime();                                 \
+        __builtin_amdgcn_sched_barrier(0);                                                          \
+        if ((threadIdx.x & 63) == 0 && blockIdx.x < kStampWgs)                                      \
+            psvo_g_stamps[k][blockIdx.x][threadIdx.x >> 6][it][i] = t_;                             \
+    } while (0)
 #else
 #define PSVO_STAMP_DECL
 #define PSVO_STAMP(i)
 #define PSVO_STAMP_FLUSH(k)
+#define PSVO_STAMP_AT(k, it, i)
 #endif
 
 }
diff --git a/proud-slam_amd/csrc/mlp_bwd.hip b/proud-slam_amd/csrc/mlp_bwd.hip
--- a/proud-slam_amd/csrc/mlp_bwd.hip
+++ b/proud-slam_amd/csrc/mlp_bwd.hip
@@ -2,6 +2,7 @@
 
 #include <cstdlib>
 
+#include "composite_ray.h"
 #include "interp_fuse.h"
 #include "mlp128_chain16.h"
 #include "mlp128_trunk_fb.h"
@@ -409,16 +410,93 @@
     const float *g_sdf, *feat, *h2;
     const int *h2_src;
 };
+template <int J, int NB>
+__device__ __forceinline__ void loss_rays(const LossFuse &lf, int r0, int r1, int64_t lo, int64_t hi, int wave,
+                                          int lane) {
+    constexpr int kWaves = kF2Threads / 64;
+    for (int rb = r0 + wave; rb <= r1; rb += kWaves * NB) {
+        int64_t r[NB];
+        RayRows rows[NB];
+#pragma unroll
+        for (int b = 0; b < NB; ++b) {
+            const int rr = rb + b * kWaves;
+            r[b] = rr <= r1 ? rr : r1;
+            rows[b] = RayRows{lo, rr <= r1 ? hi : lo, false};
+        }
+        composite_loss_rays<J, true, NB>(r, lane, lf.s_max, lf.tr, lf.max_depth, lf.offsets, lf.ray_ns, lf.z_vals,
+                                         lf.z_stride, lf.rank_ray, lf.gt_rgb, lf.gt_depth, lf.sdf_s, lf.rgb_s, lf.coef,
+                                         nullptr, nullptr, nullptr, lf.g_sdf_s, lf.g_rgb_s, 0, lf.cidx, rows);
+    }
+}
+__device__ __forceinline__ void loss_prologue_a(const LossFuse &lf, int64_t lo, int64_t hi) {
+    const int lane = threadIdx.x & 63;
+    const int wave = __builtin_amdgcn_readfirstlane(threadIdx.x >> 6);
+    const int r0 = __builtin_amdgcn_readfirstlane(lf.ray_of[lo]);
+    const int r1 = __builtin_amdgcn_readfirstlane(lf.ray_of[hi - 1]);
+    switch (composite_loss_j(lf.s_max)) {
+    case 2: loss_rays<2, 1>(lf, r0, r1, lo, hi, wave, lane); break;
+    case 4: loss_rays<4, 1>(lf, r0, r1, lo, hi, wave, lane); break;
+    case 8: loss_rays<8, 1>(lf, r0, r1, lo, hi, wave, lane); break;
+    default: loss_rays<0, 1>(lf, r0, r1, lo, hi, wave, lane); break;
+    }
+}
+__device__ __forceinline__ void loss_prologue_b(const LossFuse &lf, int64_t lo, int64_t hi) {
+    const float cfs = lf.coef[2], csdf = lf.coef[3];
+    for (int64_t j0 = lo + threadIdx.x; j0 < hi; j0 += 2 * kF2Threads) {
+        const int64_t jj[2] = {j0, j0 + kF2Threads < hi ? j0 + kF2Threads : j0};
+        int src[2], ray[2], off[2];
+        int64_t orig[2];
+        float p[2], z[2], d[2];
+#pragma unroll
+        for (int k = 0; k < 2; ++k) {
+            src[k] = lf.src[jj[k]];
+            ray[k] = lf.ray_of[jj[k]];
+        }
+#pragma unroll
+        for (int k = 0; k < 2; ++k) {
+            p[k] = lf.sdf_s[src[k]];
+            off[k] = lf.offsets[ray[k]];
+            orig[k] = lf.rank_ray[ray[k]];
+        }
+#pragma unroll
+        for (int k = 0; k < 2; ++k) {
+            z[k] = lf.z_vals[(int64_t)ray[k] * lf.z_stride + (src[k] - off[k])];
+            d[k] = lf.gt_depth[orig[k]];
+        }
+#pragma unroll
+        for (int k = 0; k < 2; ++k) {
+            const float gsdf = crit_grad(cfs, csdf, crit_terms(z[k], p[k], d[k], lf.tr, lf.max_depth));
+            lf.g_sdf_s[jj[k]] = comp_gsdf(0.f, 0.f, 1.f, false, p[k], lf.tr, gsdf);
+        }
+    }
+}
+
 template <bool W, bool H2>
 __global__ __launch_bounds__(kF2Threads, 1) void k_mlp_bwd3(int64_t m, const float *__restrict__ img, Bwd3Src src,
                                                             DwGrid g, float *__restrict__ slabs, InterpFuse ip,
                                                             const int *__restrict__ m_dev, TrunkSrc tk,
-                                                            InterpFuse ip_b, BwdSplitCost cost) {
+                                                            InterpFuse ip_b, BwdSplitCost cost, LossFuse lf) {
     static_assert(W, "the two-class launch is a training launch");
     const int n_wg = gridDim.x, b = blockIdx.x;
     if (m_dev) m = __builtin_amdgcn_readfirstlane(*m_dev);
     const int64_t m_b = __builtin_amdgcn_readfirstlane(*tk.m_dev);
     const int n_a = bwd_split_na((m + kU - 1) / kU, (m_b + kU - 1) / kU, n_wg, cost);
+    if (lf.sdf_s != nullptr) {
+        const bool cls_a = b < n_a;
+        const int64_t mc = cls_a ? m : m_b, units = (mc + kU - 1) / kU;
+        const int64_t wg = cls_a ? b : b - n_a, n = cls_a ? n_a : n_wg - n_a;
+        const int64_t s0 = units * wg / n * kU, s1e = units * (wg + 1) / n * kU, s1 = s1e < mc ? s1e : mc;
+        const int64_t base = cls_a ? 0 : lf.cap;
+        PSVO_STAMP_AT(cls_a ? 1 : 2, 0, 14);
+        if (s0 < s1) {
+            if (cls_a)
+                loss_prologue_a(lf, s0, s1);
+            else
+                loss_prologue_b(lf, base + s0, base + s1);
+        }
+        __syncthreads();
+        PSVO_STAMP_AT(cls_a ? 1 : 2, 0, 15);
+    }
     if (b < n_a)
         mlp_bwd3_body<true>(b, n_a, b, m, img, src, g, slabs, ip);
     else
@@ -442,6 +520,10 @@
     *slab_floats = off;
 }
 
+}
+
+bool dec128_bwd_one_launch(int64_t m, bool counts_on_device, bool two_launch) {
+    return m > 0 && bwd3_grid(m) >= 2 && counts_on_device && !two_launch;
 }
 
 int64_t dec128_workspace_floats(int64_t m) {
@@ -505,21 +587,23 @@
     const bool trunk_last = tb && m > 0;
     bool bound = false;
     const hipEvent_t bind_ev = bind_env ? dfeat_ready : nullptr;
-    const bool one_launch = trunk_last && grid >= 2 && m_dev && !tb->two_launch;
+    const bool one_launch = trunk_last && dec128_bwd_one_launch(m, m_dev != nullptr, tb->two_launch);
+    PSVO_REQUIRE(!tb || !tb->loss || one_launch, "mlp_bwd: the loss pass runs inside the one-launch backward only");
     if (one_launch) {
         PSVO_REQUIRE(!tb->h2 || tb->src, "mlp_bwd: the trunk's h2 rows need their source index");
         cnt_a = m_dev;
         cnt_b = tb->m_dev;
         const TrunkSrc tk{tb->m_dev, tb->g_sdf, tb->feat, tb->h2, tb->src};
         const InterpFuse ip_a = ip ? *ip : InterpFuse{}, ip_b = tb->ip ? *tb->ip : InterpFuse{};
+        const LossFuse lf = tb->loss ? *tb->loss : LossFuse{};
         constexpr int kLdsAb = kLdsBwd3 > kLdsTrunk ? kLdsBwd3 : kLdsTrunk;
         psvo::StopBind sb(bind_ev);
         if (tb->h2)
             launch_lds<k_mlp_bwd3<true, true>>(dim3(grid), dim3(kF2Threads), kLdsAb, st, m, images, src, g, slabs,
-                                               ip_a, m_dev, tk, ip_b, cost);
+                                               ip_a, m_dev, tk, ip_b, cost, lf);
         else
             launch_lds<k_mlp_bwd3<true, false>>(dim3(grid), dim3(kF2Threads), kLdsAb, st, m, images, src, g, slabs,
-                                                ip_a, m_dev, tk, ip_b, cost);
+                                                ip_a, m_dev, tk, ip_b, cost, lf);
         bound = sb.consumed();
         const int rc = check_launch("mlp_bwd3 (both classes)");
         if (rc) return rc;
diff --git a/proud-slam_amd/csrc/psvo_common.h b/proud-slam_amd/csrc/psvo_common.h
--- a/proud-slam_amd/csrc/psvo_common.h
+++ b/proud-slam_amd/csrc/psvo_common.h
@@ -279,6 +279,16 @@
                    const float *gx, float *grad_o, float *grad_d, const int *offsets2 = nullptr,
                    const float *t2 = nullptr, const float *gx2 = nullptr);
 
+struct LossFuse {
+    int s_max, z_stride;
+    float tr, max_depth;
+    const int *offsets, *ray_ns, *rank_ray, *cidx, *ray_of, *src;
+    const float *z_vals, *gt_rgb, *gt_depth, *sdf_s, *rgb_s, *coef;
+    float *g_sdf_s, *g_rgb_s;
+    int64_t cap;
+};
+bool dec128_bwd_one_launch(int64_t m, bool counts_on_device, bool two_launch);
+
 struct TrunkBwd {
     const int *m_dev;
     const float *g_sdf, *feat;
@@ -286,6 +296,7 @@
     const float *h2 = nullptr;
     const int *src = nullptr;
     bool two_launch = false;
+    const LossFuse *loss = nullptr;
 };
 
 struct BwdSplitCost {
diff --git a/proud-slam_amd/psvo/_lib.py b/proud-slam_amd/psvo/_lib.py
--- a/proud-slam_amd/psvo/_lib.py
+++ b/proud-slam_amd/psvo/_lib.py
@@ -71,6 +71,7 @@
     "psvo_engine_free": (None, [_vp]),
     "psvo_engine_set_timing": (_i32, [_vp, _i32]),
     "psvo_engine_set_paths": (_i32, [_vp, _i32]),
+    "psvo_engine_loss_in_bwd": (_i32, [_vp]),
     "psvo_engine_select_stats": (_i32, [_vp, _vp, _vp, _i32]),
     "psvo_engine_gate_stream": (_i32, [_vp, _vp]),
     "psvo_debug_set_lookback": (_i32, [_i32, _i32, _i32]),
diff --git a/proud-slam_amd/psvo/engine.py b/proud-slam_amd/psvo/engine.py
--- a/proud-slam_amd/psvo/engine.py
+++ b/proud-slam_amd/psvo/engine.py
@@ -300,9 +300,13 @@
                self.step_no, 1 if marked else 0)
 
     PATH_QUERY_SPLIT, PATH_PADDED, PATH_DENSE_DECODER, PATH_INTERP_PASS, PATH_BWD_TWO_LAUNCH = 1, 2, 4, 8, 16
+    PATH_LOSS_PASS = 32
 
     def set_paths(self, paths):
         L.call("psvo_engine_set_paths", self.handle, int(paths))
+
+    def loss_in_bwd(self):
+        return bool(L.lib().psvo_engine_loss_in_bwd(self.handle))
 
     def select_stats(self, reset=False):
         out = (ctypes.c_int64 * 5)()
```

After: 6.617 million (median of 6 runs). 1.1% higher.
